# PrimeIntellect-ai/protocol

Hardware: AMD Instinct MI355X
Metric: task x worker pair-evals/sec (full-swarm match) (higher is better)
Workload: dtype u64

## Files before the change

protocol_amd/csrc/pm_device.h:

```cpp
#ifndef PM_DEVICE_H
#define PM_DEVICE_H

#include <hip/hip_runtime.h>
#include <stdint.h>

#include "pm_engine.h"

namespace pm {

static constexpr double PM_RAD = 3.14159265358979323846 / 180.0;
static constexpr uint64_t PM_KEY_NOLOC = 0x7FEFFFFFFFFFFFFFull;
static constexpr double PM_A_MAX_SAFE = 1.0 - 1.0 / 1048576.0;
static constexpr double PM_A_CHORD_MIN = 1.3e-6;
static constexpr uint32_t PM_CARVE_SLOTS = 8192;
static constexpr uint32_t PM_CARVE_PART = 64;
static constexpr uint32_t PM_CARVE_SEL_CAP = 256;
static constexpr uint32_t PM_CARVE_SLOT_BITS = 13;
static constexpr uint32_t PM_CARVE_BIG_SLOTS = 262144;
static constexpr uint32_t PM_CARVE_SLOT_BITS_BIG = 18;
static constexpr uint32_t PM_CARVE_SLOT_BITS_MEM = 21;
static constexpr double PM_TIE_BAND = 1.0 / 68719476736.0;
static constexpr double PM_TIE_BAND_BIG = 1.0 / 2147483648.0;
static constexpr double PM_TIE_BAND_MEM = 1.0 / 268435456.0;
static constexpr uint32_t PM_PROP_ROW = 96;
// ... 23 lines not shown
#define PM_STREAM_PROP_WAVES_N 4
#endif
static constexpr uint32_t PM_STREAM_PROP_WAVES = PM_STREAM_PROP_WAVES_N;
static constexpr uint32_t PM_STREAM_SLW_TREQ = PM_STREAM_TP;
static constexpr uint32_t PM_STREAM_SLW_PAY = PM_STREAM_TP + 1;
static constexpr size_t PM_STREAM_LDS_BYTES = PM_CARVE_LDS_BYTES + size_t(PM_STREAM_TP) * 4 + 128;
enum { SC_CLAIM = 0,
       SC_QUIT = 16,
       SC_DROP = 32,
       SC_ROWS = 48,
       SC_LET_BE = 53,
       SC_GAVE_UP = 49,
       SC_FINISH = 50,
       SC_FINISH_TICKET = 52,
       SC_TRACE = 51,
       SC_BATCHES = 54
};
static constexpr uint32_t PM_STREAM_TRACE_CAP = 1u << 17;
enum { SROW_NONE = 0, SROW_BITMAP = 1, SROW_WALK = 2, SROW_SWEEP = 3 };

struct CompatArgs {
  uint32_t W, n_cfgs, model_words;
  const uint32_t *flags, *gpu_count, *gpu_mem, *gpu_cls, *cpu_cores, *ram, *storage;
  const pm_config_row* cfgs;
  const pm_gpu_alt_row* alts;
  const uint32_t* model_bits;
  uint64_t* compat;
};

enum : uint32_t {
  REP_WHY = 0,
  REP_IDLE = PM_WHY_N,
  REP_GROUPS,
  REP_MEMBERS,
  REP_NO_TASK,
  REP_TASKS,
  REP_STRIDE = 16
};

struct ReportArgs {
  CompatArgs c;
  const int32_t* group_of;
  const uint32_t *g_cfg, *g_n, *g_task, *live_bits;
  uint32_t G;
  const uint64_t *tmask, *tlive;
  const uint32_t* tprefix;
  uint32_t t_lo, t_cap;
  uint32_t* out;
  uint32_t *running, *workers, *allowed;
};

struct SpreadArgs {
  const uint32_t *g_n, *g_off, *members, *slot_of_row, *small, *big;
  uint32_t n_small, n_big, W;
  const uint32_t *flags, *addr_rank;
  const double *lat, *lon, *coslat;
  pm_group_spread_row* out;
};
enum : uint32_t { SPC_GROUPS = 0, SPC_MEASURED = 1, SPC_HIST = 2, SPC_N = 2 + PM_SPREAD_BUCKETS, SPC_STRIDE = 8 };
enum : uint32_t { SPV_MAX_DIAMETER = 0, SPV_MAX_HOP = 1, SPV_SUM_DIAMETER = 2, SPV_SUM_RING = 3 };
struct SpreadCfgAcc {
  uint32_t cnt[SPC_STRIDE];
  unsigned long long v[4];
};

static constexpr uint32_t PM_NEAR_CAP = 2u * PM_NEAR_MAX_K;
struct NearArgs {
  CompatArgs c;
  const int32_t* group_of;
  const double *lat, *lon, *coslat;
  const pm_near_query* q;
  uint32_t n_q, pool, k;
  pm_near_row* rows;
  uint32_t* workers;
  double* km;
};

struct ClaimArgs {
  uint32_t R;
  const uint32_t* rows;
  const int32_t* group_of;
  const uint32_t *g_n, *g_off, *g_task;
  const uint64_t* g_id;
  uint32_t* g_task_next;
  const uint32_t* chosen;
  const uint32_t* rank_in_group;
  const uint32_t* by_rank;
  const uint64_t* t_live;
  const uint32_t* t_prefix;
  pm_assignment* table;
  uint32_t* task_col;
  pm_assignment* h_table;
  uint32_t* h_gtask;
};

struct MatchPrepArgs {
  uint32_t W, G;
  const int32_t* group_of;
  const uint32_t *g_cfg, *g_n, *g_off, *members, *addr_rank, *g_task;
  uint64_t* sel;
  uint32_t *first, *count;
  uint32_t *rank_in_group, *by_rank;
  uint32_t* g_task_next;
};

struct RowUpdateArgs {
  uint32_t n;
  const double *lat_in, *lon_in;
  const uint32_t* u32_in;
  uint32_t *flags, *gpu_count, *gpu_mem, *gpu_cls, *cpu_cores, *ram, *storage, *addr_rank, *site;
  double *lat, *lon, *coslat;
  double *ux, *uy, *uz;
};

enum { CARVE_MODE_FORM = 0, CARVE_MODE_MERGE = 1 };
enum { CARVE_STATE_RUNNING = 0, CARVE_STATE_DONE = 1, CARVE_STATE_UNCERTAIN = 2, CARVE_STATE_OVERFLOW = 3,
       CARVE_STATE_ABORTED = 4 };
enum {
  CARVE_F_INIT = 1u << 0,
  CARVE_F_RUN = 1u << 1,
  CARVE_F_ALL = 1u << 2,
  CARVE_F_PROPS = 1u << 3,
  CARVE_F_EXTPREP = 1u << 4
};
struct CarveStatus {
  uint32_t state;
  uint32_t stop_ci;
  uint32_t n_groups;
  uint32_t n_members;
  uint32_t steps_total;
  uint32_t n_eligible;
  uint32_t cur_ci;
  uint32_t n_list;
  unsigned long long cand_sum;
  uint32_t prop_k;
  uint32_t prop_limit;
  uint32_t n_seeds;
  uint32_t total_available;
  uint32_t fast_steps;
  uint32_t slow_steps;
  uint32_t n_solo;
  uint32_t n_props;
  uint32_t g_lo, g_hi;
  uint32_t n_batches;
  uint32_t n_void;
  uint32_t why[8];
  uint32_t stream_timeouts;
  uint32_t stream_tickets;
  uint32_t stream_switches;
  uint32_t stream_listed;
  uint32_t stream_pre_used;
  uint32_t stream_pre_lost;
  uint32_t stream_refreshes;
  uint32_t _pad_sr;
  uint32_t cell_g;
  uint32_t n_indexed;
  uint32_t pruned_batches;
  uint32_t prune_fallbacks;
#ifdef PM_BATCH_LOG
  uint32_t blog_n;
  uint32_t blog[3 * 512];
#endif
  unsigned long long prop_keys;
  unsigned long long prof[64];
};

struct alignas(16) BatchDesc {
  uint32_t planned;
  uint32_t ci0;
  uint32_t total_available;
  uint32_t valid;
  uint32_t none;
  uint32_t ci, n_list, prop_k, prop_limit, n_seeds;
  uint32_t cell_g;
};

struct CarveArgs {
  uint32_t mode;
  uint32_t W;
  uint32_t proximity;
  uint32_t debug_uncertain_every;
  const uint32_t* wflags;
  const double *lat, *lon, *coslat;
  const double *ux, *uy, *uz;
  const uint32_t* site;
  const uint64_t* compat;
  int32_t* group_of;
  uint32_t* order;
  uint32_t n_order;
  uint32_t _pad2;
  double *c_lat, *c_lon, *c_cos;
  double *c_ux, *c_uy, *c_uz;
  uint32_t* c_site;
  uint64_t* c_compat;
  uint64_t *alive_g, *loc_g;
  double *cc_lat, *cc_lon, *cc_cos;
  double *cc_ux, *cc_uy, *cc_uz;
  uint32_t* cc_site;
  uint32_t* slot_pos;
  uint32_t* slot_wid;
  uint64_t* bits_scratch;
  uint64_t* keys;
  uint32_t bits_stride;
  uint32_t _pad0;
  uint64_t* prop;
  uint64_t* seed_map;
  uint32_t* seed_prefix;
  uint32_t* seed_slots;
  uint32_t count_keys, _pad_ck;
  uint32_t* prep_block_counts;
  uint32_t* prep_counts;
  BatchDesc* desc;
  uint64_t* alive_snap;
  uint32_t _pad_sp;
  uint32_t debug_mem_above;
  uint32_t* cell_cnt;
  uint32_t* cell_start;
  uint32_t *pos_cell, *pos_rank;
  uint32_t* cs_of_pos;
  uint32_t* cs_slot;
  double *cs_ux, *cs_uy, *cs_uz;
  uint32_t* cs_site;
  uint32_t prune_mode;
  uint32_t prune_factor;
  uint32_t walk_cap_div, _pad_w;
  uint32_t stream, stream_tag0;
  double* c_pack;
  double* cs_pack;
  uint64_t* cfgbits;
  unsigned long long* stream_sq;
  unsigned long long* stream_row_lo;
  unsigned long long* stream_row_hi;
  uint32_t* stream_ctl;
  uint32_t stream_la, stream_row_spins;
  uint32_t stream_la_div;
  uint32_t debug_abort_after;
  unsigned long long id_state;
  uint32_t id_g0, stage_m0;
  uint32_t stage_cap_g, stage_cap_m;
  uint32_t *stage_cfg, *stage_n, *stage_off, *stage_mem;
  unsigned long long* g_id_out;
  uint32_t* g_task_out;
  CarveStatus* h_status;
  unsigned long long* stream_trace;
  uint32_t n_avail, start_ci;
  uint32_t avail_cfg[PM_MAX_CONFIGS];
  uint32_t min_size[PM_MAX_CONFIGS];
  uint32_t max_size[PM_MAX_CONFIGS];
  uint32_t *g_cfg, *g_n, *g_off, *members;
  uint32_t cap_groups, cap_members;
  CarveStatus* status;
};

void launch_compat(const CompatArgs& a, hipStream_t s);
void launch_explain(const CompatArgs& p, const uint32_t* rows, uint32_t n, uint32_t stride, uint32_t* why_out, hipStream_t s);
void launch_config_report(const ReportArgs& a, uint32_t max_blocks, hipStream_t s);
void launch_task_report(const ReportArgs& a, uint32_t max_blocks, hipStream_t s);
void launch_group_spread(const SpreadArgs& a, hipStream_t s);
void launch_config_spread(const pm_group_spread_row* rows, const uint32_t* row_cfg, uint32_t n_rows, uint32_t n_cfgs,
                          SpreadCfgAcc* out, uint32_t max_blocks, hipStream_t s);
void launch_nearest(const NearArgs& a, hipStream_t s);
void launch_geo(const double* lat, const double* lon, double* coslat, double* ux, double* uy, double* uz, uint32_t W,
                hipStream_t s);
void launch_triad(const double* b, const double* c, double* a, size_t n, hipStream_t s);
#ifdef PM_ROW_BENCH
hipError_t launch_row_bench(const CarveArgs* d_args, uint32_t seed, uint32_t ci, uint32_t reps, uint32_t mode, unsigned long long* d_out, hipStream_t s);
#endif
void launch_row_network_test(const uint64_t* keys, const uint32_t* sites, uint32_t n_waves, uint32_t n_per_wave, uint32_t slot_bits,
                             uint64_t ulps, uint32_t upto, uint64_t* rows_out, uint32_t* mismatches, hipStream_t s);
static constexpr uint32_t PM_DK_WORDS = 20;
void launch_distance_key_test(const double* in, const double* geo, uint32_t n, uint32_t mode, double* out, hipStream_t s);
void launch_update_rows(const RowUpdateArgs& a, hipStream_t s);
void launch_worker_selector(const int32_t* group_of, const uint32_t* g_cfg, uint32_t R, const uint32_t* rows,
                            uint64_t* sel, hipStream_t s);
void launch_eligible_selector(const uint32_t* wflags, const int32_t* group_of, const uint64_t* compat,
                              uint64_t enabled, uint32_t W, const uint8_t* shard, uint32_t my_rank, uint64_t* sel,
                              hipStream_t s);
void launch_chooser_rank(const int32_t* group_of, const uint64_t* g_id, const uint32_t* count, uint32_t R,
                         const uint32_t* rows, uint64_t seed, uint32_t* rank, hipStream_t s);
void launch_table_scatter(const pm_assignment* x, const uint32_t* xrow, uint32_t W, pm_assignment* table,
                          uint32_t* task_col, uint32_t* g_task_next, const uint64_t* t_live, const uint32_t* t_prefix,
                          hipStream_t s);
void launch_group_rank(const int32_t* group_of, const uint32_t* g_n, const uint32_t* g_off, const uint32_t* members,
                       const uint32_t* addr_rank, uint32_t W, uint32_t* rank_in_group, uint32_t* by_rank,
                       hipStream_t s);
void launch_claim_publish(const ClaimArgs& a, hipStream_t s);
void launch_match_prep(const MatchPrepArgs& a, hipStream_t s);
void launch_build_planes(const uint64_t* col_mask, uint32_t n_cols, uint32_t c_begin, uint32_t c_end, uint32_t stride,
                         uint32_t n_planes, uint64_t* planes, hipStream_t s);
void launch_pair_sweep(int variant, const uint64_t* row_sel, uint32_t R, const uint64_t* col_mask,
                       const uint64_t* planes, uint32_t c_begin, uint32_t c_end, uint32_t stride, uint32_t n_planes,
                       uint32_t* first, uint32_t* count, hipStream_t s, bool inited = false);
void launch_pair_select(int variant, const uint64_t* row_sel, uint32_t R, const uint64_t* col_mask,
                        const uint64_t* planes, uint32_t c_begin, uint32_t c_end, uint32_t stride, uint32_t n_planes,
                        const uint32_t* rank, uint32_t* out, hipStream_t s);
void launch_task_prefix(const uint64_t* live, uint32_t w_begin, uint32_t w_end, uint32_t* prefix, hipStream_t s);
void launch_task_delete(const uint32_t* slots, uint32_t n, uint64_t* tmask, uint64_t* live, uint64_t* planes,
                        uint32_t stride, uint32_t n_planes, hipStream_t s);
void launch_task_intern(const uint64_t* tmask, const uint64_t* live, uint32_t u_begin, uint32_t u_end, uint64_t valid,
                        uint64_t* keys, uint32_t n_slots, uint32_t* vals, uint32_t* counter_and_overflow, uint64_t* umask,
                        uint32_t cap_u, hipStream_t s);
void launch_task_compact_class(const uint32_t* first_c, const uint32_t* count_c, const uint64_t* tmask, uint64_t valid,
                               const uint64_t* keys, const uint32_t* vals, uint32_t n_slots, uint32_t u_begin,
                               uint32_t u_end, const uint64_t* live, const uint32_t* prefix, uint32_t* first_out,
                               uint32_t* count_out, hipStream_t s);
void launch_task_compact(const uint32_t* first_u, const uint32_t* count_u, uint32_t u_begin, uint32_t u_end,
                         const uint64_t* live, const uint32_t* prefix, uint32_t* first_out, uint32_t* count_out,
                         hipStream_t s);
void launch_newest(const int64_t* created_at, const uint64_t* live, uint32_t t_begin, uint32_t t_end,
                   uint32_t* idx_by_block, long long* val_by_block, uint32_t n_blocks, hipStream_t s);
void launch_group_ids(uint64_t* g_id, uint32_t* g_task, uint32_t n, uint64_t rng_state, hipStream_t s);
hipError_t carve_kernels_init();
hipError_t launch_carve(const CarveArgs* d_args, uint32_t flags, uint32_t start_ci, size_t lds_bytes, hipStream_t s);
uint32_t launch_carve_prep(const CarveArgs* d_args, uint32_t W, hipStream_t s);
hipError_t launch_carve_args_put(const CarveArgs& a, CarveArgs* d_args, hipStream_t s);
uint32_t launch_carve_elig(CarveArgs* d_args, const CarveArgs* put, uint32_t W, uint32_t n_bound, uint32_t index_min, uint32_t start_ci,
                           bool fresh, uint32_t n_groups0, uint32_t n_members0, hipStream_t s);
void launch_carve_apply(const CarveArgs* d_args, uint32_t W, hipStream_t s);
void launch_carve_propose(const CarveArgs* d_args, uint32_t W, hipStream_t s);
hipError_t launch_carve_stream(const CarveArgs* d_args, uint32_t start_ci, uint32_t n_prop_wgs, hipStream_t s);
void launch_scatter_const(uint32_t* dst, const uint32_t* idx, uint32_t n, uint32_t v, hipStream_t s);
void launch_scatter_pairs(uint32_t* dst, const uint32_t* pairs, uint32_t n, hipStream_t s);
void launch_merge_place(const CarveArgs* d_args, uint32_t n_order, uint32_t n_groups0, uint32_t n_members0, uint32_t steps0,
                        hipStream_t s);

}
#endif
```

protocol_amd/csrc/pm_engine.cpp:

```cpp
#include <hip/hip_runtime.h>

#include <algorithm>
#include <atomic>
#include <cmath>
#include <chrono>
#include <cstdio>
#include <cstdlib>
#include <cstring>
#include <functional>
#include <memory>
#include <mutex>
#include <string>
#include <thread>
#include <unordered_map>
#include <vector>

#include "pm_device.h"
#include "pm_engine.h"
#include "pm_internal.h"
#include "pm_members.h"

namespace pm {

static thread_local std::string g_last_error;

int32_t set_error(int32_t code, const std::string& msg) {
  g_last_error = msg;
  return code;
}

#define HIPCHK(expr)                                                                                   \
  do {                                                                                                 \
    hipError_t e_ = (expr);                                                                            \
    if (e_ != hipSuccess)                                                                              \
      return set_error(PM_ENODEV, std::string(#expr) + ": " + hipGetErrorString(e_));                  \
  } while (0)

#include "pm_engine_types.inc"
}

using namespace pm;

namespace pm {
struct FormRun;
}

#include "pm_engine_state.inc"

namespace pm {

#include "pm_engine_groups.inc"
#include "pm_engine_carve.inc"
#include "pm_engine_match.inc"
#include "pm_engine_merge.inc"
}


extern "C" {

const char* pm_last_error(void) { return pm::g_last_error.c_str(); }

void pm_engine_config_default(pm_engine_config* c) {
  if (!c) return;
  std::memset(c, 0, sizeof(*c));
  c->abi_version = PM_ABI_VERSION;
  c->device = 0;
  c->proximity_enabled = 1;
  c->switching_enabled = 1;
  c->prefer_larger_groups = 1;
  c->chooser = PM_CHOOSE_FIRST;
  c->group_id_seed = 1;
}

int32_t pm_engine_create(const pm_engine_config* cfg, pm_engine** out) {
  if (!cfg || !out) return set_error(PM_EINVAL, "null argument");
  if (cfg->abi_version != PM_ABI_VERSION) return set_error(PM_EINVAL, "ABI version mismatch");
  if (cfg->carve_variant != 0 && cfg->carve_variant != 1 && cfg->carve_variant != 3)
    return set_error(PM_EINVAL, "carve_variant: 0 (streaming carve), 1 (exact sweep only) or 3 (batch pipeline); 2 and 4 were removed");
  int n_dev = 0;
  if (hipGetDeviceCount(&n_dev) != hipSuccess || n_dev <= 0)
    return set_error(PM_ENODEV, "no HIP device visible: the matching engine needs an MI355X (gfx950); there is no CPU fallback");
  if (cfg->device < 0 || cfg->device >= n_dev) return set_error(PM_EINVAL, "device ordinal out of range");
  HIPCHK(hipSetDevice(cfg->device));
  hipDeviceProp_t prop;
  HIPCHK(hipGetDeviceProperties(&prop, cfg->device));
  if (std::strncmp(prop.gcnArchName, "gfx950", 6) != 0)
    return set_error(PM_ENODEV, std::string("device is ") + prop.gcnArchName + ", kernels are built for gfx950 only");
  HIPCHK(carve_kernels_init());
  pm_engine* e = new (std::nothrow) pm_engine();
  if (!e) return set_error(PM_ENOMEM, "out of host memory");
  e->cfg = *cfg;
  e->id_rng = cfg->group_id_seed;
  if (const char* v = getenv("PM_PRUNE_MODE")) {
    if (v[0] >= '0' && v[0] <= '3' && !v[1]) e->prune_mode = uint32_t(v[0] - '0');
  }
  if (const char* v = getenv("PM_WALK_CAP_DIV")) {
    const long f = atol(v);
    if (f > 0 && f < 1000) e->walk_cap_div = uint32_t(f);
  }
  if (const char* v = getenv("PM_PRUNE_FACTOR")) {
    const long f = atol(v);
    if (f > 0 && f < (1l << 30)) e->prune_factor = uint32_t(f);
  }
  if (const char* v = getenv("PM_STREAM_WGS")) {
    const long f = atol(v);
    if (f > 0 && f < 4096) e->stream_wgs_env = uint32_t(f);
  }
  if (const char* v = getenv("PM_STREAM_ROW_SPINS")) {
    const long f = atol(v);
    if (f > 0 && f < (1l << 24)) e->stream_row_spins_env = uint32_t(f);
  }
  if (const char* v = getenv("PM_STREAM_LA_DIV")) {
    const long f = atol(v);
    if (f > 0 && f < 4096) e->stream_la_div_env = uint32_t(f);
  }
  if (const char* v = getenv("PM_MERGE_STREAM_MIN")) {
    const long f = atol(v);
    if (f >= 2 && f <= (1l << 30)) e->merge_stream_min = uint32_t(f);
  }
  if (const char* v = getenv("PM_STREAM_LA")) {
    const long f = atol(v);
    if (f > 0 && f <= long(PM_STREAM_LA_MAX)) e->stream_la_env = uint32_t(f);
  }
  {
    int cus = 0;
    if (hipDeviceGetAttribute(&cus, hipDeviceAttributeMultiprocessorCount, cfg->device) == hipSuccess && cus > 0)
      e->n_cus = uint32_t(cus);
  }
  if (hipStreamCreateWithFlags(&e->stream, hipStreamNonBlocking) != hipSuccess) {
    delete e;
    return set_error(PM_ENODEV, "hipStreamCreate failed");
  }
  e->stream_owned = e->stream;
  for (auto& ev : e->ev)
    if (hipEventCreate(&ev) != hipSuccess) {
      delete e;
      return set_error(PM_ENODEV, "hipEventCreate failed");
    }
  for (auto& ev : e->kev)
    if (hipEventCreate(&ev) != hipSuccess) {
      delete e;
      return set_error(PM_ENODEV, "hipEventCreate failed");
    }
  if (hipEventCreateWithFlags(&e->ev_groups, hipEventDisableTiming) != hipSuccess) {
    delete e;
    return set_error(PM_ENODEV, "hipEventCreate failed");
  }
  *out = e;
  return PM_OK;
}

void pm_engine_destroy(pm_engine* e) {
  if (!e) return;
  (void)hipSetDevice(e->cfg.device);
  (void)hipStreamSynchronize(e->stream);
  e->d_cfgs.release(); e->d_alts.release(); e->d_model_bits.release();
  e->d_flags.release(); e->d_gpu_count.release(); e->d_gpu_mem.release(); e->d_gpu_cls.release();
  e->d_cpu_cores.release(); e->d_ram.release(); e->d_storage.release(); e->d_addr_rank.release();
  e->d_lat.release(); e->d_lon.release(); e->d_coslat.release(); e->d_compat.release();
  e->d_ux.release(); e->d_uy.release(); e->d_uz.release();
  for (int k = 0; k < 3; ++k) { e->d_c_u[k].release(); e->d_cc_u[k].release(); }
  e->d_tmask.release(); e->d_tplanes.release(); e->d_created.release(); e->d_tlive.release(); e->d_tprefix.release();
  e->d_first_c.release(); e->d_count_c.release(); e->d_tdel.release();
  e->d_group_of.release(); e->d_g_cfg.release(); e->d_g_n.release(); e->d_g_off.release();
  e->d_g_task.release(); e->d_g_task_next.release(); e->d_members.release(); e->d_by_rank.release();
  e->d_rank_in_group.release(); e->d_g_id.release();
  e->d_order.release(); e->d_c_lat.release(); e->d_c_lon.release(); e->d_c_cos.release();
  e->d_cc_lat.release(); e->d_cc_lon.release(); e->d_cc_cos.release(); e->d_slot_pos.release(); e->d_slot_wid.release();
  e->d_site.release(); e->d_c_site.release(); e->d_cc_site.release(); e->d_prop.release(); e->d_seed_map.release(); e->d_seed_prefix.release(); e->d_seed_slots.release(); e->d_prep_block_counts.release(); e->d_prep_counts.release();
  e->d_c_compat.release(); e->d_keys.release(); e->d_bits.release(); e->d_status.release(); e->d_carve_args.release();
  e->d_m_cfg.release(); e->d_m_n.release(); e->d_m_off.release(); e->d_m_members.release();
  e->d_cfgbits.release(); e->d_stream_sq.release(); e->d_stream_row_lo.release(); e->d_stream_row_hi.release();
  e->d_stream_ctl.release(); e->d_stream_trace.release();
  e->d_sel.release(); e->d_wplanes.release(); e->d_sel_perm.release();
  e->d_first.release(); e->d_count.release(); e->d_rank.release(); e->d_chosen.release(); e->d_perm.release();
  e->d_table.release(); e->d_task_col.release(); e->d_shard.release(); e->d_own_rows.release(); e->d_xrow.release();
  e->d_sel_own.release(); e->d_table_x.release(); e->d_row_stage.release(); if (e->h_row_pin) (void)hipHostFree(e->h_row_pin); if (e->ev_row_stage) (void)hipEventDestroy(e->ev_row_stage); e->d_nb_idx.release(); e->d_nb_val.release();
  if (e->h_gstage) (void)hipHostFree(e->h_gstage);
  if (e->h_status) (void)hipHostFree(e->h_status);
  for (int k = 0; k < 2; ++k) {
    if (e->h_delta_pin[k]) (void)hipHostFree(e->h_delta_pin[k]);
    e->d_delta[k].release();
  }
  if (e->h_gtask_pinned) (void)hipHostFree(e->h_gtask_pinned);
  if (e->ev_groups) (void)hipEventDestroy(e->ev_groups);
  for (PubTable& t : e->pub)
    if (t.words.load()) (void)hipHostFree(t.words.load());
  for (uint64_t* q : e->pub_retired) (void)hipHostFree(q);
  for (auto& ev : e->ev)
    if (ev) (void)hipEventDestroy(ev);
  for (auto& ev : e->kev)
    if (ev) (void)hipEventDestroy(ev);
  for (hipEvent_t x : e->prop_ev) (void)hipEventDestroy(x);
  if (e->stream_owned) (void)hipStreamDestroy(e->stream_owned);
  e->d_cell_cnt.release(); e->d_cell_start.release(); e->d_pos_cell.release(); e->d_pos_rank.release();
  e->d_cs_of_pos.release(); e->d_cs_slot.release(); e->d_cs_site.release();
  for (auto& u : e->d_cs_u) u.release();
  e->d_c_pack.release();
  e->d_cs_pack.release();
  e->d_desc.release(); e->d_snap.release(); e->d_ikeys.release(); e->d_umask.release(); e->d_ivals.release();
  e->d_rep_rows.release(); e->d_rep_why.release(); e->d_rep_flags.release(); e->d_rep_live.release(); e->d_rep_g.release();
  e->d_rep_tprefix.release(); e->d_rep_cnt.release(); e->d_rep_task.release(); e->d_rep_gof.release();
  e->d_spr_idx.release(); e->d_spr_rows.release(); e->d_spr_acc.release();
  e->d_near_q.release(); e->d_near_out.release();
  delete e->form;
  delete e;
}

int32_t pm_set_configs(pm_engine* e, const pm_config_row* cfgs, uint32_t n_cfgs, const pm_gpu_alt_row* alts,
                       uint32_t n_alts) {
  if (!e || (n_cfgs && !cfgs) || (n_alts && !alts)) return set_error(PM_EINVAL, "null argument");
  if (n_cfgs > PM_MAX_CONFIGS) return set_error(PM_EINVAL, "more than PM_MAX_CONFIGS configurations");
  for (uint32_t i = 0; i < n_cfgs; ++i) {
    if (cfgs[i].max_group_size < cfgs[i].min_group_size)
      return set_error(PM_EINVAL, "Plugin configuration is invalid (max_group_size < min_group_size)");
    if (cfgs[i].min_group_size == 0)
      return set_error(PM_EINVAL, "min_group_size == 0 is rejected (the reference would form empty groups forever)");
    if (uint64_t(cfgs[i].alt_begin) + cfgs[i].alt_count > n_alts)
      return set_error(PM_ERANGE, "alternative range outside the alt table");
  }
  std::lock_guard<std::mutex> lk(e->mu);
  if (e->dist_phase != 0) return set_error(PM_ESTATE, "a stepwise tick is in progress");
  HIPCHK(hipSetDevice(e->cfg.device));
  e->cfgs.assign(cfgs, cfgs + n_cfgs);
  e->alts.assign(alts, alts + n_alts);
  int32_t rc = upload(e->d_cfgs, e->cfgs.data(), e->cfgs.size(), e->stream);
  if (rc) return rc;
  rc = upload(e->d_alts, e->alts.data(), e->alts.size(), e->stream);
  if (rc) return rc;
  HIPCHK(e->d_model_bits.ensure(1));
  HIPCHK(hipStreamSynchronize(e->stream));
  e->have_cfgs = true;
  e->compat_dirty = true;
  e->tplanes_dirty = true;
  return PM_OK;
}

int32_t pm_set_model_table(pm_engine* e, const uint32_t* bits, uint32_t n_rows, uint32_t n_classes) {
  if (!e || (n_rows && n_classes && !bits)) return set_error(PM_EINVAL, "null argument");
  std::lock_guard<std::mutex> lk(e->mu);
  HIPCHK(hipSetDevice(e->cfg.device));
  const size_t words = size_t(n_rows) * ((n_classes + 31u) / 32u);
  e->model_bits.assign(bits, bits + words);
  e->model_rows = n_rows;
  e->model_classes = n_classes;
  e->cls_check_dirty = true;
  int32_t rc = upload(e->d_model_bits, e->model_bits.data(), words, e->stream);
  if (rc) return rc;
  HIPCHK(hipStreamSynchronize(e->stream));
  e->compat_dirty = true;
  return PM_OK;
}

int32_t pm_set_enabled_mask(pm_engine* e, uint64_t enabled) {
  if (!e) return set_error(PM_EINVAL, "null argument");
  std::lock_guard<std::mutex> lk(e->mu);
  if (e->dist_phase != 0) return set_error(PM_ESTATE, "a stepwise tick is in progress");
  e->enabled = enabled;
  return PM_OK;
}

#include "pm_engine_workers.inc"
#include "pm_engine_tasks.inc"
// ... 10 lines not shown
```

protocol_amd/csrc/pm_engine_carve.inc:

```
static int32_t ensure_compat(pm_engine* e, hipEvent_t end_ev = nullptr) {
  if (!e->have_cfgs || !e->have_workers) return set_error(PM_ESTATE, "configs and workers must be uploaded first");
  {
    int32_t rcf = sync_flags(e);
    if (rcf) return rcf;
  }
  if (!e->compat_dirty) return PM_OK;
  for (const pm_gpu_alt_row& a : e->alts)
    if ((a.flags & PM_G_MODEL) && a.model_row >= e->model_rows)
      return set_error(PM_ESTATE, "a GPU alternative names a model row but pm_set_model_table was not called");
  if (e->model_rows && e->cls_check_dirty)
    for (uint32_t w = 0; w < e->W; ++w)
      if ((e->h_flags[w] & PM_W_GPU_MODEL) && e->h_gpu_cls[w] >= e->model_classes)
        return set_error(PM_ERANGE, "worker gpu_model_class outside the model table");
  e->cls_check_dirty = false;
  HIPCHK(e->d_compat.ensure(std::max<size_t>(e->W, 1)));
  CompatArgs a{};
  a.W = e->W;
  a.n_cfgs = uint32_t(e->cfgs.size());
  a.model_words = (e->model_classes + 31u) / 32u;
  a.flags = e->d_flags.p;
  a.gpu_count = e->d_gpu_count.p;
  a.gpu_mem = e->d_gpu_mem.p;
  a.gpu_cls = e->d_gpu_cls.p;
  a.cpu_cores = e->d_cpu_cores.p;
// ... 50 lines not shown
  HIPCHK(e->d_c_lat.ensure(cap));
  HIPCHK(e->d_c_lon.ensure(cap));
  HIPCHK(e->d_c_cos.ensure(cap));
  HIPCHK(e->d_cc_lat.ensure(cap));
  HIPCHK(e->d_cc_lon.ensure(cap));
  HIPCHK(e->d_cc_cos.ensure(cap));
  for (int k = 0; k < 3; ++k) {
    HIPCHK(e->d_c_u[k].ensure(cap));
    HIPCHK(e->d_cc_u[k].ensure(cap));
  }
  HIPCHK(e->d_c_compat.ensure(cap));
  HIPCHK(e->d_keys.ensure(cap));
  HIPCHK(e->d_slot_pos.ensure(cap));
  HIPCHK(e->d_slot_wid.ensure(cap));
  HIPCHK(e->d_c_site.ensure(cap));
  HIPCHK(e->d_cc_site.ensure(cap));
  {
    HIPCHK(e->d_prop.ensure((size_t(PM_PROP_MAX_SEEDS) + 64) * PM_PROP_ROW));
    HIPCHK(e->d_seed_map.ensure((cap + 63) / 64 + 64));
    HIPCHK(e->d_seed_prefix.ensure((cap + 63) / 64 + 64));
    HIPCHK(e->d_seed_slots.ensure(size_t(PM_PROP_MAX_SEEDS) + 128));
    HIPCHK(e->d_prep_block_counts.ensure(((cap + 255) / 256 + 1) * PM_MAX_CONFIGS));
    HIPCHK(e->d_prep_counts.ensure(PM_MAX_CONFIGS + 8));
  }
  HIPCHK(e->d_status.ensure(1));
  HIPCHK(e->d_carve_args.ensure(1));
  HIPCHK(e->d_desc.ensure(1));
  const uint32_t stride = uint32_t((cap + 63) / 64);
  HIPCHK(e->d_bits.ensure(size_t(stride) * 4));
  HIPCHK(e->d_snap.ensure(stride));
  if (stream) {
    HIPCHK(e->d_c_pack.ensure(cap * 4));
    HIPCHK(e->d_cs_pack.ensure(cap * 4));
    HIPCHK(e->d_cfgbits.ensure(size_t(stride) * PM_MAX_CONFIGS));
    HIPCHK(e->d_stream_ctl.ensure(PM_STREAM_CTL_WORDS));
    if (!e->d_stream_sq.p) {
      HIPCHK(e->d_stream_sq.ensure(PM_STREAM_SQ));
      HIPCHK(e->d_stream_row_lo.ensure(size_t(PM_STREAM_RQ) * 64));
      HIPCHK(e->d_stream_row_hi.ensure(size_t(PM_STREAM_RQ) * 64));
      e->stream_seq = 0;
    }
  }
  if (mode == CARVE_MODE_FORM && e->prune_mode && e->cfg.proximity_enabled) {
    if (!e->d_cell_cnt.p) {
      HIPCHK(e->d_cell_cnt.ensure(PM_CELL_TABLE));
      HIPCHK(hipMemsetAsync(e->d_cell_cnt.p, 0, e->d_cell_cnt.cap * sizeof(uint32_t), e->stream));
    }
    if (!e->d_cell_start.p) {
      HIPCHK(e->d_cell_start.ensure(PM_CELL_TABLE + 384));
      HIPCHK(hipMemsetAsync(e->d_cell_start.p, 0, e->d_cell_start.cap * sizeof(uint32_t), e->stream));
    }
    HIPCHK(e->d_pos_cell.ensure(cap));
    HIPCHK(e->d_pos_rank.ensure(cap));
    HIPCHK(e->d_cs_of_pos.ensure(cap));
    HIPCHK(e->d_cs_slot.ensure(cap));
    HIPCHK(e->d_cs_site.ensure(cap));
    for (auto& u : e->d_cs_u) HIPCHK(u.ensure(cap));
  }
  std::memset(a, 0, sizeof(*a));
  a->mode = mode;
  a->W = e->W;
  a->proximity = e->cfg.proximity_enabled;
  a->debug_uncertain_every = e->cfg.debug_uncertain_every;
  a->wflags = e->d_flags.p;
  a->lat = e->d_lat.p;
  a->lon = e->d_lon.p;
  a->coslat = e->d_coslat.p;
  a->ux = e->d_ux.p;
  a->uy = e->d_uy.p;
  a->uz = e->d_uz.p;
  a->compat = e->d_compat.p;
  a->group_of = e->d_group_of.p;
  a->order = e->d_order.p;
  a->n_order = n_order;
  a->c_lat = e->d_c_lat.p;
  a->c_lon = e->d_c_lon.p;
  a->c_cos = e->d_c_cos.p;
  a->c_ux = e->d_c_u[0].p;
  a->c_uy = e->d_c_u[1].p;
  a->c_uz = e->d_c_u[2].p;
  a->c_compat = e->d_c_compat.p;
  a->alive_g = e->d_bits.p;
  a->loc_g = e->d_bits.p + stride;
  a->cc_lat = e->d_cc_lat.p;
  a->cc_lon = e->d_cc_lon.p;
  a->cc_cos = e->d_cc_cos.p;
  a->cc_ux = e->d_cc_u[0].p;
  a->cc_uy = e->d_cc_u[1].p;
  a->cc_uz = e->d_cc_u[2].p;
  a->keys = e->d_keys.p;
  a->slot_pos = e->d_slot_pos.p;
  a->slot_wid = e->d_slot_wid.p;
  a->site = e->d_site.p;
  a->c_site = e->d_c_site.p;
  a->cc_site = e->d_cc_site.p;
  a->prop = e->d_prop.p;
  a->seed_map = e->d_seed_map.p;
  a->seed_prefix = e->d_seed_prefix.p;
  a->seed_slots = e->d_seed_slots.p;
  a->count_keys = e->cfg.time_proposer ? 1u : 0u;
  a->prep_block_counts = e->d_prep_block_counts.p;
  a->prep_counts = e->d_prep_counts.p;
  a->bits_scratch = e->d_bits.p + size_t(stride) * 2;
  a->bits_stride = stride;
  a->status = e->d_status.p;
  a->desc = e->d_desc.p;
  a->alive_snap = e->d_snap.p;
  a->debug_mem_above = e->debug_mem_above;
  if (mode == CARVE_MODE_FORM && e->prune_mode && e->cfg.proximity_enabled) {
    a->prune_mode = e->prune_mode;
    a->prune_factor = e->prune_factor;
    a->walk_cap_div = e->walk_cap_div;
    a->cell_cnt = e->d_cell_cnt.p;
    a->cell_start = e->d_cell_start.p;
    a->pos_cell = e->d_pos_cell.p;
    a->pos_rank = e->d_pos_rank.p;
    a->cs_of_pos = e->d_cs_of_pos.p;
    a->cs_slot = e->d_cs_slot.p;
    a->cs_site = e->d_cs_site.p;
    a->cs_ux = e->d_cs_u[0].p;
    a->cs_uy = e->d_cs_u[1].p;
    a->cs_uz = e->d_cs_u[2].p;
  }
  if (stream) {
    a->stream = 1;
    a->cc_lat = a->c_lat;
    a->cc_lon = a->c_lon;
    a->cc_cos = a->c_cos;
    a->cc_ux = a->c_ux;
    a->cc_uy = a->c_uy;
    a->cc_uz = a->c_uz;
    a->cc_site = a->c_site;
    a->slot_wid = a->order;
    a->bits_scratch = e->d_bits.p;
    a->loc_g = e->d_bits.p + stride;
    a->alive_g = e->d_bits.p + size_t(stride) * 2;
    a->cfgbits = e->d_cfgbits.p;
    a->c_pack = e->d_c_pack.p;
    a->cs_pack = e->d_cs_pack.p;
    a->stream_sq = (unsigned long long*)e->d_stream_sq.p;
    a->stream_row_lo = (unsigned long long*)e->d_stream_row_lo.p;
    a->stream_row_hi = (unsigned long long*)e->d_stream_row_hi.p;
    a->stream_ctl = e->d_stream_ctl.p;
#if defined(PM_CARVE_PROF) || defined(PM_ROW_REC)
    HIPCHK(e->d_stream_trace.ensure(size_t(PM_STREAM_TRACE_CAP) * 2));
    a->stream_trace = (unsigned long long*)e->d_stream_trace.p;
#endif
#ifdef PM_ROW_REC
    HIPCHK(hipMemsetAsync(e->d_stream_trace.p, 0, size_t(PM_STREAM_TRACE_CAP) * 16, e->stream));
#endif
    a->stream_la = e->stream_la_env;
    a->stream_la_div = e->stream_la_div_env;
    a->stream_row_spins = e->stream_row_spins_env;
    a->debug_abort_after = e->debug_abort_after;
  }
  return PM_OK;
}

static int32_t host_resolve_form_step(pm_engine* e, uint32_t cfg, CarveStatus* st) {
  int32_t rc = pull_compat(e);
  if (rc) return rc;
  std::vector<int32_t> group_of(e->W);
  if (e->W) {
    HIPCHK(hipMemcpyAsync(group_of.data(), e->d_group_of.p, size_t(e->W) * 4, hipMemcpyDeviceToHost, e->stream));
    HIPCHK(hipStreamSynchronize(e->stream));
  }
  const pm_config_row& c = e->cfgs[cfg];
  std::vector<uint32_t> compat;
  size_t total_available = 0;
  for (uint32_t w = 0; w < e->W; ++w) {
    const uint32_t f = e->h_flags[w];
    if (!((f & PM_W_HEALTHY) && (f & PM_W_HAS_P2P) && group_of[w] < 0)) continue;
    ++total_available;
    if ((e->h_compat[w] >> cfg) & 1ull) compat.push_back(w);
  }
  if (total_available < c.min_group_size || compat.size() < c.min_group_size || compat.empty())
    return set_error(PM_ESTATE, "host resolve: nothing to carve (state mismatch)");
  uint32_t seed = compat[0];
  bool seed_loc = false;
  for (uint32_t w : compat)
    if (e->h_flags[w] & PM_W_HAS_LOC) {
      seed = w;
      seed_loc = true;
      break;
    }
  std::vector<uint32_t> rest;
  for (uint32_t w : compat)
    if (w != seed) rest.push_back(w);
  if (seed_loc && e->cfg.proximity_enabled) {
    std::vector<double> d(e->W, 0.0);
    for (uint32_t w : rest)
      d[w] = (e->h_flags[w] & PM_W_HAS_LOC) ? host_distance(e->h_lat[seed], e->h_lon[seed], e->h_lat[w], e->h_lon[w])
                                            : 1.7976931348623157e308;
    std::stable_sort(rest.begin(), rest.end(), [&](uint32_t a, uint32_t b) { return d[a] < d[b]; });
  }
  std::vector<uint32_t> members{seed};
  for (uint32_t w : rest) {
    if (members.size() >= c.max_group_size) break;
    members.push_back(w);
  }
  if (members.size() < c.min_group_size) return set_error(PM_ESTATE, "host resolve: group below min size");
  const uint32_t g = st->n_groups, off = st->n_members, n = uint32_t(members.size());
  if (g >= e->d_g_cfg.cap || off + n > e->d_members.cap) return set_error(PM_ENOMEM, "group arrays overflow");
  HIPCHK(hipMemcpyAsync(e->d_g_cfg.p + g, &cfg, 4, hipMemcpyHostToDevice, e->stream));
  HIPCHK(hipMemcpyAsync(e->d_g_n.p + g, &n, 4, hipMemcpyHostToDevice, e->stream));
  HIPCHK(hipMemcpyAsync(e->d_g_off.p + g, &off, 4, hipMemcpyHostToDevice, e->stream));
  HIPCHK(hipMemcpyAsync(e->d_members.p + off, members.data(), size_t(n) * 4, hipMemcpyHostToDevice, e->stream));
  for (uint32_t w : members) group_of[w] = int32_t(g);
  HIPCHK(hipMemcpyAsync(e->d_group_of.p, group_of.data(), size_t(e->W) * 4, hipMemcpyHostToDevice, e->stream));
  HIPCHK(hipStreamSynchronize(e->stream));
  st->n_groups += 1;
  st->n_members += n;
  st->n_solo += n == 1 ? 1u : 0u;
  st->steps_total += 1;
  return PM_OK;
}

static int32_t absorb_groups(pm_engine* e) {
  if (!e->absorb_pending) return PM_OK;
  HIPCHK(hipEventSynchronize(e->ev_groups));
  const uint32_t g0 = e->ab_g0, ng = e->ab_g1 - e->ab_g0, m0 = e->ab_m0;
  const uint32_t *g_cfg = e->ab_cfg_p, *g_n = e->ab_n_p, *g_off = e->ab_off_p, *members = e->ab_mem_p;
  if (e->groups.capacity() < e->groups.size() + ng) e->groups.reserve(std::max(e->groups.size() + ng, e->groups.capacity() * 2));
  for (uint32_t k = 0; k < ng; ++k) {
    Group gr;
    gr.id = splitmix64_next(&e->id_rng);
    gr.cfg = g_cfg[k];
    gr.task = PM_NONE;
    gr.task_uid = 0;
    gr.members.assign(members + (g_off[k] - m0), members + (g_off[k] - m0) + g_n[k]);
    for (uint32_t w : gr.members) e->h_group_of[w] = int32_t(g0 + k);
    log_group_event(e, PM_GROUP_CREATED, gr);
    e->groups.push_back(std::move(gr));
  }
  e->absorb_pending = false;
  return PM_OK;
}

#define ABSORB_PENDING(e)                 \
  do {                                    \
    int32_t rc_abs_ = absorb_groups(e);   \
    if (rc_abs_) return rc_abs_;          \
  } while (0)

static void host_mark(const char* what) {
  static const bool on = [] { const char* v = getenv("PM_TRACE_HOST"); return v && *v == '1'; }();
  if (!on) return;
  static const auto t0 = std::chrono::steady_clock::now();
  const double us = std::chrono::duration<double, std::micro>(std::chrono::steady_clock::now() - t0).count();
  fprintf(stderr, "[pm host] %10.1f us  %s\n", us, what);
}

struct FormRun {
  CarveArgs a;
  CarveStatus st;
  std::vector<uint32_t> avail;
  uint32_t g0 = 0, m0 = 0, start_ci = 0;
  size_t lds = 0;
  bool use_props = false;
  bool nothing = false;
  uint32_t n_bound = 0;
  uint32_t n_elig_hint = 0;
  bool stream = false;
  uint32_t stream_wgs = 0;
  bool rearmed = false;
  uint32_t stage_cap = 0;
  bool args_pending = false;
};

static int32_t launch_propose_timed(pm_engine* e, const CarveArgs* d_args, uint32_t n_bound, hipStream_t s);

static int32_t form_setup_args(pm_engine* e, FormRun* r);

static int32_t form_queue_init(pm_engine* e, FormRun* r, bool fresh = false) {
  fresh = fresh && r->use_props;
  if (!fresh) HIPCHK(hipMemcpyAsync(e->d_status.p, &r->st, sizeof(r->st), hipMemcpyHostToDevice, e->stream));
  if (r->use_props) {
    if (!r->stream) HIPCHK(hipMemsetAsync(e->d_desc.p, 0, sizeof(BatchDesc), e->stream));
    const uint32_t index_min = !r->a.prune_mode ? 0u : r->a.prune_mode >= 2u ? 1u : PM_CELL_AUTO_N;
    if (r->stream) {
      if (e->stream_seq == 0 || e->stream_seq >= 127) {
        HIPCHK(hipMemsetAsync(e->d_stream_sq.p, 0, size_t(PM_STREAM_SQ) * 8, e->stream));
        HIPCHK(hipMemsetAsync(e->d_stream_row_lo.p, 0, size_t(PM_STREAM_RQ) * 64 * 8, e->stream));
        HIPCHK(hipMemsetAsync(e->d_stream_row_hi.p, 0, size_t(PM_STREAM_RQ) * 64 * 8, e->stream));
        e->stream_seq = 0;
      }
      e->stream_seq += 1;
      const uint32_t tag0 = e->stream_seq << 25;
      if (r->a.stream_tag0 != tag0) {
        r->a.stream_tag0 = tag0;
        if (!r->args_pending)
          HIPCHK(hipMemcpyAsync(&e->d_carve_args.p->stream_tag0, &r->a.stream_tag0, sizeof(uint32_t), hipMemcpyHostToDevice, e->stream));
      }
    }
    e->tick_carve_launches += launch_carve_elig(e->d_carve_args.p, r->args_pending ? &r->a : nullptr, e->W, r->n_bound,
                                                r->n_elig_hint >= index_min ? index_min : 0u, r->start_ci, fresh, r->st.n_groups,
                                                r->st.n_members, e->stream);
    r->args_pending = false;
    host_mark("form: eligible list queued");
    if (r->stream) {
      HIPCHK(launch_carve_stream(e->d_carve_args.p, r->start_ci, r->stream_wgs, e->stream));
      e->tick_carve_launches += 2;
      return PM_OK;
    }
    e->tick_carve_launches += launch_carve_prep(e->d_carve_args.p, r->n_bound, e->stream);
    HIPCHK(hipGetLastError());
  } else
    HIPCHK(launch_carve(e->d_carve_args.p, CARVE_F_INIT | CARVE_F_RUN | CARVE_F_ALL, r->start_ci, r->lds, e->stream));
  e->tick_carve_launches++;
  return PM_OK;
}

static int32_t form_begin(pm_engine* e, FormRun* r, hipEvent_t begin_ev = nullptr) {
  int32_t rc = absorb_groups(e);
  if (rc) return rc;
  rc = ensure_compat(e);
  if (rc) return rc;
  rc = push_groups(e);
  if (rc) return rc;
  available_order(e->cfgs.data(), uint32_t(e->cfgs.size()), e->enabled, &r->avail);
  r->g0 = e->d_n_groups;
  r->m0 = e->d_n_members;
  r->start_ci = 0;
  r->nothing = r->avail.empty() || e->W == 0;
  if (r->nothing) return PM_OK;
  if (e->h_group_of.size() == e->W && e->h_flags.size() == e->W) {
    const int32_t* const gof = e->h_group_of.data();
    const uint32_t* const fl = e->h_flags.data();
    const uint32_t need = PM_W_HEALTHY | PM_W_HAS_P2P;
    uint32_t nb = 0, ne = 0;
    for (uint32_t w = 0; w < e->W; ++w) {
      const uint32_t un = uint32_t(gof[w]) >> 31;
      nb += un;
      ne += un & uint32_t((fl[w] & need) == need);
    }
    r->n_bound = nb;
    r->n_elig_hint = ne;
  } else {
    r->n_bound = uint32_t(std::count_if(e->h_group_of.begin(), e->h_group_of.end(), [](int32_t g) { return g < 0; }));
    r->n_elig_hint = r->n_bound;
  }
  if (e->h_group_of.size() != e->W) r->n_bound = r->n_elig_hint = e->W;
  if (r->n_bound == 0) r->n_bound = 1;
  r->st = CarveStatus{};
  r->st.state = CARVE_STATE_RUNNING;
  r->st.n_groups = r->g0;
  r->st.n_members = r->m0;
  r->use_props = e->cfg.carve_variant != 1 && e->cfg.proximity_enabled;
  r->stream = r->use_props && e->cfg.carve_variant == 0 && r->n_bound <= PM_CARVE_BIG_SLOTS &&
              !e->debug_mem_above;
  host_mark("form: begin (host mirrors counted)");
  rc = form_setup_args(e, r);
  if (rc) return rc;
  host_mark("form: arguments queued");
  if (begin_ev && r->args_pending) {
    e->k_carve_begin = begin_ev;
  } else {
    HIPCHK(hipEventRecord(e->kev[2], e->stream));
    e->k_carve_begin = e->kev[2];
  }
  return form_queue_init(e, r, true);
}

static int32_t form_setup_args(pm_engine* e, FormRun* r) {
  CarveArgs& a = r->a;
  int32_t rc = fill_carve_args(e, &a, CARVE_MODE_FORM, 0, r->stream);
  if (rc) return rc;
  if (r->stream) {
    uint32_t wgs = e->stream_wgs_env ? e->stream_wgs_env : r->n_elig_hint / 64u + 48u;
    const uint32_t max_wgs = e->n_cus > 8u ? e->n_cus - 4u : 4u;
    r->stream_wgs = std::max(1u, std::min(wgs, max_wgs));
    a.stream_tag0 = ((e->stream_seq == 0 || e->stream_seq >= 127) ? 1u : e->stream_seq + 1u) << 25;
    a.id_state = e->id_rng;
    a.id_g0 = r->g0;
    a.stage_m0 = r->m0;
    a.g_id_out = (unsigned long long*)e->d_g_id.p;
    a.g_task_out = e->d_g_task.p;
    r->stage_cap = std::max<uint32_t>(r->n_bound, 1u);
    const size_t need = size_t(4) * r->stage_cap;
    if (e->h_gstage_cap < need) {
      HIPCHK(hipStreamSynchronize(e->stream));
      if (e->h_gstage) (void)hipHostFree(e->h_gstage);
      e->h_gstage = nullptr;
      e->h_gstage_cap = 0;
      const size_t cap = std::max<size_t>(need, size_t(4) * std::max<uint32_t>(e->W, 1));
      HIPCHK(hipHostMalloc((void**)&e->h_gstage, cap * sizeof(uint32_t)));
      e->h_gstage_cap = cap;
    }
    if (!e->h_status) HIPCHK(hipHostMalloc((void**)&e->h_status, sizeof(CarveStatus)));
    a.stage_cap_g = a.stage_cap_m = r->stage_cap;
    a.stage_cfg = e->h_gstage;
    a.stage_n = e->h_gstage + r->stage_cap;
    a.stage_off = e->h_gstage + size_t(2) * r->stage_cap;
    a.stage_mem = e->h_gstage + size_t(3) * r->stage_cap;
    a.h_status = e->h_status;
    e->h_status->state = 0xFFFFFFFFu;
  }
  a.n_avail = uint32_t(r->avail.size());
  for (size_t i = 0; i < r->avail.size(); ++i) {
    a.avail_cfg[i] = r->avail[i];
    a.min_size[i] = e->cfgs[r->avail[i]].min_group_size;
    a.max_size[i] = e->cfgs[r->avail[i]].max_group_size;
  }
  a.g_cfg = e->d_g_cfg.p;
  a.g_n = e->d_g_n.p;
  a.g_off = e->d_g_off.p;
  a.members = e->d_members.p;
  a.cap_groups = uint32_t(std::min<size_t>(e->d_g_cfg.cap, 0xFFFFFFFFu));
  a.cap_members = uint32_t(std::min<size_t>(e->d_members.cap, 0xFFFFFFFFu));
  bool in_lds;
  r->lds = carve_lds_bytes(a.bits_stride, &in_lds);
  r->args_pending = r->use_props;
  if (!r->args_pending) HIPCHK(launch_carve_args_put(a, e->d_carve_args.p, e->stream));
  return PM_OK;
}

static int32_t launch_propose_timed(pm_engine* e, const CarveArgs* d_args, uint32_t n_bound, hipStream_t s) {
  if (!e->cfg.time_proposer) {
    launch_carve_propose(d_args, n_bound, s);
    return PM_OK;
  }
  while (e->prop_ev.size() < e->prop_ev_used + 2) {
    hipEvent_t x = nullptr;
    HIPCHK(hipEventCreate(&x));
    e->prop_ev.push_back(x);
  }
  HIPCHK(hipEventRecord(e->prop_ev[e->prop_ev_used], s));
  launch_carve_propose(d_args, n_bound, s);
  HIPCHK(hipEventRecord(e->prop_ev[e->prop_ev_used + 1], s));
  e->prop_ev_used += 2;
  return PM_OK;
}

static int32_t form_queue_pairs(pm_engine* e, FormRun* r, uint32_t count) {
  for (uint32_t k = 0; k < count; ++k) {
    int32_t rc = launch_propose_timed(e, e->d_carve_args.p, r->n_bound, e->stream);
    if (rc) return rc;
    HIPCHK(launch_carve(e->d_carve_args.p, CARVE_F_RUN | CARVE_F_PROPS | CARVE_F_EXTPREP, 0, r->lds, e->stream));
    e->tick_carve_launches += 2u + launch_carve_prep(e->d_carve_args.p, r->n_bound, e->stream);
  }
  return PM_OK;
}

static int32_t form_poll(pm_engine* e, FormRun* r) {
  for (;;) {
    HIPCHK(hipEventRecord(e->kev[3], e->stream));
    HIPCHK(hipMemcpyAsync(&r->st, e->d_status.p, sizeof(r->st), hipMemcpyDeviceToHost, e->stream));
    HIPCHK(hipStreamSynchronize(e->stream));
    {
      float ms = 0;
      HIPCHK(hipEventElapsedTime(&ms, e->k_carve_begin ? e->k_carve_begin : e->kev[2], e->kev[3]));
      e->k_ms_carve += ms;
      HIPCHK(hipEventRecord(e->kev[2], e->stream));
      e->k_carve_begin = e->kev[2];
      for (size_t k = 0; k + 1 < e->prop_ev_used; k += 2) {
        HIPCHK(hipEventElapsedTime(&ms, e->prop_ev[k], e->prop_ev[k + 1]));
        e->k_ms_propose += ms;
      }
      e->prop_ev_used = 0;
    }
    if (r->st.state == CARVE_STATE_OVERFLOW) return set_error(PM_ENOMEM, "carve: group arrays overflow");
    if (r->st.state == CARVE_STATE_ABORTED) {
      if (!r->stream) return set_error(PM_ENODEV, "carve: a hand-shake inside the validator timed out");
      e->tick_stream_aborts++;
      r->rearmed = true;
      r->stream = false;
      int32_t rca = form_setup_args(e, r);
      if (rca) return rca;
      r->start_ci = r->st.stop_ci;
      r->st.state = CARVE_STATE_RUNNING;
      rca = form_queue_init(e, r);
      if (rca) return rca;
      return PM_OK;
    }
    if (r->st.state != CARVE_STATE_UNCERTAIN) return PM_OK;
    int32_t rc = host_resolve_form_step(e, r->avail[r->st.stop_ci], &r->st);
    if (rc) return rc;
    e->tick_host_resolved++;
    r->rearmed = true;
    r->start_ci = r->st.stop_ci;
    r->st.state = CARVE_STATE_RUNNING;
    rc = form_queue_init(e, r);
    if (rc) return rc;
  }
}

static int32_t form_finish(pm_engine* e, FormRun* r, uint32_t* n_formed, bool defer_absorb, bool have_event = false) {
  if (n_formed) *n_formed = 0;
  if (r->nothing) return PM_OK;
  const CarveStatus& st = r->st;
  e->tick_fast_steps += st.fast_steps;
  e->tick_carve_steps += st.steps_total;
  e->tick_cand_sum += st.cand_sum;
  e->tick_props += r->stream && !st.n_props ? st.stream_tickets : st.n_props;
  e->tick_prop_keys += st.prop_keys;
  e->tick_stream_timeouts += st.stream_timeouts;
  e->tick_stream_tickets += st.stream_tickets;
  std::memcpy(e->carve_prof, st.prof, sizeof(st.prof));
  for (int k = 0; k < 8; ++k) e->carve_why[k] = st.why[k];
  e->carve_why[8] = st.n_batches;
  e->carve_why[9] = st.n_void;
  e->carve_why[10] = st.pruned_batches;
  e->carve_why[11] = st.prune_fallbacks;
  e->carve_why[12] = st.cell_g;
  e->carve_why[13] = st.n_indexed;
  e->carve_why[14] = r->stream ? 1u : 0u;
  e->carve_why[15] = st.stream_tickets;
  e->carve_why[16] = st.stream_timeouts;
  e->carve_why[17] = st.stream_switches;
  e->carve_why[18] = st.stream_listed;
  e->carve_why[19] = r->stream_wgs;
  e->carve_why[20] = e->tick_stream_aborts;
  e->carve_why[21] = st.slow_steps;
  e->carve_why[22] = st.stream_pre_used;
  e->carve_why[23] = st.stream_pre_lost;
  e->carve_why[24] = st.stream_refreshes;
#ifdef PM_BATCH_LOG
  e->blog.assign(st.blog, st.blog + 3 * std::min<uint32_t>(st.blog_n, 512u));
#endif

  const uint32_t g0 = r->g0, m0 = r->m0, g1 = st.n_groups, m1 = st.n_members;
  if (g1 > g0) {
    const uint32_t ng = g1 - g0, nm = m1 - m0;
    const bool staged = r->stream && !r->rearmed && ng <= r->stage_cap && nm <= r->stage_cap;
    if (staged) {
      e->ab_cfg_p = e->h_gstage;
      e->ab_n_p = e->h_gstage + r->stage_cap;
      e->ab_off_p = e->h_gstage + size_t(2) * r->stage_cap;
      e->ab_mem_p = e->h_gstage + size_t(3) * r->stage_cap;
      if (!have_event) HIPCHK(hipEventRecord(e->ev_groups, e->stream));
    } else {
      const size_t need = size_t(3) * ng + nm;
      if (e->h_gstage_cap < need) {
        if (e->h_gstage) (void)hipHostFree(e->h_gstage);
        e->h_gstage = nullptr;
        e->h_gstage_cap = 0;
        const size_t cap = std::max<size_t>(need, size_t(4) * std::max<uint32_t>(e->W, 1));
        HIPCHK(hipHostMalloc((void**)&e->h_gstage, cap * sizeof(uint32_t)));
        e->h_gstage_cap = cap;
      }
      uint32_t* st_cfg = e->h_gstage;
      HIPCHK(hipMemcpyAsync(st_cfg, e->d_g_cfg.p + g0, size_t(ng) * 4, hipMemcpyDeviceToHost, e->stream));
      HIPCHK(hipMemcpyAsync(st_cfg + ng, e->d_g_n.p + g0, size_t(ng) * 4, hipMemcpyDeviceToHost, e->stream));
      HIPCHK(hipMemcpyAsync(st_cfg + 2 * size_t(ng), e->d_g_off.p + g0, size_t(ng) * 4, hipMemcpyDeviceToHost, e->stream));
      HIPCHK(hipMemcpyAsync(st_cfg + 3 * size_t(ng), e->d_members.p + m0, size_t(nm) * 4, hipMemcpyDeviceToHost, e->stream));
      e->ab_cfg_p = st_cfg;
      e->ab_n_p = st_cfg + ng;
      e->ab_off_p = st_cfg + 2 * size_t(ng);
      e->ab_mem_p = st_cfg + 3 * size_t(ng);
      HIPCHK(hipEventRecord(e->ev_groups, e->stream));
      host_mark("form: group copies queued");
      launch_group_ids(e->d_g_id.p + g0, e->d_g_task.p + g0, ng, e->id_rng, e->stream);
      HIPCHK(hipGetLastError());
    }
    e->absorb_pending = true;
    e->ab_g0 = g0;
    e->ab_g1 = g1;
    e->ab_m0 = m0;
    e->ab_m1 = m1;
    e->ab_solo = st.n_solo;
    e->d_n_groups = g1;
    e->d_n_members = m1;
    if (!defer_absorb) {
      int32_t rc = absorb_groups(e);
      if (rc) return rc;
    }
  }
  if (n_formed) *n_formed = g1 - g0;
  return PM_OK;
}

static int32_t run_form_wait(pm_engine* e, FormRun& r) {
  int32_t rc = PM_OK;
  if (!r.nothing) {
    uint32_t batch = e->form_rounds_hint ? e->form_rounds_hint + 1u : r.a.n_avail + 3u;
    for (uint32_t spins = 0;; ++spins) {
      if (spins > 4096u + e->W / 8u) return set_error(PM_ENODEV, "carve made no progress");
      if (r.use_props && !r.stream) {
        rc = form_queue_pairs(e, &r, batch);
        if (rc) return rc;
      }
      host_mark("form: carve queued");
      rc = form_poll(e, &r);
      if (rc) return rc;
      host_mark("form: status back");
      if (r.st.state == CARVE_STATE_DONE) break;
      if (r.st.state != CARVE_STATE_RUNNING || !r.use_props) return set_error(PM_ENODEV, "carve kernel did not complete");
      if (r.stream) return set_error(PM_ENODEV, "streaming carve did not complete");
      batch = 8u;
    }
  }
  if (!r.nothing && r.use_props && !r.stream) e->form_rounds_hint = r.st.n_batches + r.st.n_void;
  return PM_OK;
}
static int32_t run_form_rest(pm_engine* e, FormRun& r, uint32_t* n_formed, bool defer_absorb) {
  int32_t rc = run_form_wait(e, r);
  if (rc) return rc;
  return form_finish(e, &r, n_formed, defer_absorb);
}

static int32_t run_form(pm_engine* e, uint32_t* n_formed, bool defer_absorb = false) {
  FormRun r;
  int32_t rc = form_begin(e, &r);
  if (rc) return rc;
  return run_form_rest(e, r, n_formed, defer_absorb);
}
```

protocol_amd/csrc/pm_engine_debug.inc:

```
int32_t pm_debug_carve_prof(pm_engine* e, unsigned long long* out, uint32_t cap) {
  if (!e || !out) return set_error(PM_EINVAL, "null argument");
  std::lock_guard<std::mutex> lk(e->mu);
  const uint32_t n = std::min<uint32_t>(cap, 32u);
  std::memcpy(out, e->carve_prof, size_t(n) * sizeof(unsigned long long));
  for (uint32_t k = 32; k < cap && k < 56; ++k) out[k] = e->carve_why[k - 32];
  for (uint32_t k = 56; k < cap && k < 88; ++k) out[k] = e->carve_prof[k - 56 + 32];
  const unsigned long long inc[9] = {e->t_lo, e->t_cap, e->T, e->t_dead, e->t_regrowths, e->t_compactions,
                                     e->groups.size(), e->n_dead_groups, e->pub_retired.size()};
  for (uint32_t k = 88; k < cap && k < 97; ++k) out[k] = inc[k - 88];
  if (cap > 97u) out[97] = e->carve_why[24];
  return PM_OK;
}

int32_t pm_debug_stream_trace(pm_engine* e, unsigned long long* out, uint32_t cap, uint32_t* n) {
  if (!e || !out || !n) return set_error(PM_EINVAL, "null argument");
  std::lock_guard<std::mutex> lk(e->mu);
  *n = 0;
  if (!e->d_stream_trace.p || !e->d_stream_ctl.p) return PM_OK;
  uint32_t cnt = 0;
  HIPCHK(hipMemcpy(&cnt, e->d_stream_ctl.p + SC_TRACE, 4, hipMemcpyDeviceToHost));
#ifdef PM_ROW_REC
  cnt = std::min<uint32_t>(cnt, std::min<uint32_t>(cap, PM_STREAM_TRACE_CAP / 8u));
  if (cnt) HIPCHK(hipMemcpy(out, e->d_stream_trace.p + PM_STREAM_TRACE_CAP, size_t(cnt) * 16, hipMemcpyDeviceToHost));
#else
  cnt = std::min<uint32_t>(cnt, std::min<uint32_t>(cap, PM_STREAM_TRACE_CAP));
  if (cnt) HIPCHK(hipMemcpy(out, e->d_stream_trace.p, size_t(cnt) * 16, hipMemcpyDeviceToHost));
#endif
  *n = cnt;
  return PM_OK;
}

int32_t pm_debug_row_records(pm_engine* e, unsigned long long* out, uint32_t cap_rows, uint32_t* n_rows) {
  if (!e || !out || !n_rows) return set_error(PM_EINVAL, "null argument");
  std::lock_guard<std::mutex> lk(e->mu);
  *n_rows = 0;
#ifdef PM_ROW_REC
  if (!e->d_stream_trace.p) return PM_OK;
  const uint32_t n = std::min<uint32_t>(cap_rows, PM_STREAM_TRACE_CAP / 8u);
  HIPCHK(hipMemcpy(out, e->d_stream_trace.p, size_t(n) * 64, hipMemcpyDeviceToHost));
  *n_rows = n;
#endif
  return PM_OK;
}
int32_t pm_debug_chain_batches(pm_engine* e, unsigned long long* out, uint32_t cap, uint32_t* n) {
  if (!e || !out || !n) return set_error(PM_EINVAL, "null argument");
  std::lock_guard<std::mutex> lk(e->mu);
  *n = 0;
#ifdef PM_ROW_REC
  if (!e->d_stream_trace.p || !e->d_stream_ctl.p) return PM_OK;
  uint32_t cnt = 0;
  HIPCHK(hipMemcpy(&cnt, e->d_stream_ctl.p + SC_BATCHES, 4, hipMemcpyDeviceToHost));
  cnt = std::min<uint32_t>(cnt, std::min<uint32_t>(cap, PM_STREAM_TRACE_CAP / 8u));
  if (cnt) HIPCHK(hipMemcpy(out, e->d_stream_trace.p + PM_STREAM_TRACE_CAP + PM_STREAM_TRACE_CAP / 2u, size_t(cnt) * 32, hipMemcpyDeviceToHost));
  *n = cnt;
#endif
  return PM_OK;
}
int32_t pm_debug_park_records(pm_engine* e, unsigned long long* out, uint32_t cap_blocks, uint32_t* n_blocks) {
  if (!e || !out || !n_blocks) return set_error(PM_EINVAL, "null argument");
  std::lock_guard<std::mutex> lk(e->mu);
  *n_blocks = 0;
#ifdef PM_ROW_REC
  if (!e->d_stream_trace.p) return PM_OK;
  const uint32_t n = std::min<uint32_t>(cap_blocks, PM_STREAM_TRACE_CAP / 32u);
  HIPCHK(hipMemcpy(out, e->d_stream_trace.p + PM_STREAM_TRACE_CAP + PM_STREAM_TRACE_CAP / 4u, size_t(n) * 64, hipMemcpyDeviceToHost));
  *n_blocks = n;
#endif
  return PM_OK;
}
int32_t pm_debug_mem_lists_above(pm_engine* e, uint32_t n) {
  if (!e) return set_error(PM_EINVAL, "null argument");
  std::lock_guard<std::mutex> lk(e->mu);
  e->debug_mem_above = n;
  return PM_OK;
}

int32_t pm_debug_stream_abort_after(pm_engine* e, uint32_t n) {
  if (!e) return set_error(PM_EINVAL, "null argument");
  std::lock_guard<std::mutex> lk(e->mu);
  e->debug_abort_after = n;
  return PM_OK;
}

int32_t pm_debug_merge_streamed(pm_engine* e, uint32_t* n) {
  if (!e || !n) return set_error(PM_EINVAL, "null argument");
  std::lock_guard<std::mutex> lk(e->mu);
  *n = e->merge_streamed;
  return PM_OK;
}

int32_t pm_debug_delta_pushes(pm_engine* e, uint32_t* n) {
  if (!e || !n) return set_error(PM_EINVAL, "null argument");
  std::lock_guard<std::mutex> lk(e->mu);
  *n = e->delta_pushes;
  return PM_OK;
}

int32_t pm_debug_prune_mode(pm_engine* e, uint32_t mode) {
  if (!e || mode > 3u) return set_error(PM_EINVAL, "prune mode 0..3");
  std::lock_guard<std::mutex> lk(e->mu);
  e->prune_mode = mode;
  return PM_OK;
}

#ifdef PM_BATCH_LOG
extern "C" int32_t pm_debug_batch_log(pm_engine* e, uint32_t* out, uint32_t cap_words, uint32_t* n_words) {
  if (!e || !out || !n_words) return set_error(PM_EINVAL, "null argument");
  std::lock_guard<std::mutex> lk(e->mu);
  *n_words = uint32_t(e->blog.size());
  std::memcpy(out, e->blog.data(), sizeof(uint32_t) * std::min<size_t>(cap_words, e->blog.size()));
  return PM_OK;
}
#endif

int32_t pm_debug_hbm_triad(pm_engine* e, uint64_t n_doubles, uint32_t reps, double* gb_per_s) {
  if (!e || !gb_per_s || !n_doubles) return set_error(PM_EINVAL, "null argument");
  std::lock_guard<std::mutex> lk(e->mu);
  HIPCHK(hipSetDevice(e->cfg.device));
  double *a = nullptr, *b = nullptr, *c = nullptr;
  HIPCHK(hipMalloc((void**)&a, n_doubles * 8));
  if (hipMalloc((void**)&b, n_doubles * 8) != hipSuccess || hipMalloc((void**)&c, n_doubles * 8) != hipSuccess) {
    (void)hipFree(a);
    if (b) (void)hipFree(b);
    return set_error(PM_ENOMEM, "triad buffers");
  }
  (void)hipMemsetAsync(b, 0, n_doubles * 8, e->stream);
  (void)hipMemsetAsync(c, 0, n_doubles * 8, e->stream);
  float best = 1e30f;
  for (uint32_t r = 0; r < reps + 1; ++r) {
    (void)hipEventRecord(e->kev[0], e->stream);
    launch_triad(b, c, a, size_t(n_doubles), e->stream);
    (void)hipEventRecord(e->kev[1], e->stream);
    (void)hipEventSynchronize(e->kev[1]);
    float ms = 0;
    (void)hipEventElapsedTime(&ms, e->kev[0], e->kev[1]);
    if (r > 0 && ms < best) best = ms;
  }
  (void)hipFree(a);
  (void)hipFree(b);
  (void)hipFree(c);
  *gb_per_s = double(n_doubles) * 24.0 / (double(best) * 1e-3) / 1e9;
  return PM_OK;
}

int32_t pm_debug_row_networks(pm_engine* e, const uint64_t* keys, const uint32_t* sites, uint32_t n_waves, uint32_t n_per_wave,
                              uint32_t slot_bits, uint64_t ulps, uint32_t upto, uint64_t* rows_out, uint32_t* mismatches) {
  if (!e || !keys || !sites || !rows_out || !mismatches || !n_waves || (n_waves & 3u) || !n_per_wave || slot_bits == 0 || slot_bits > 24)
    return set_error(PM_EINVAL, "null argument");
  std::lock_guard<std::mutex> lk(e->mu);
  HIPCHK(hipSetDevice(e->cfg.device));
  const size_t nk = size_t(n_waves) * n_per_wave, ns = size_t(1) << slot_bits;
  uint64_t *d_k = nullptr, *d_rows = nullptr;
  uint32_t *d_s = nullptr, *d_m = nullptr;
  int32_t rc = PM_OK;
  if (hipMalloc((void**)&d_k, nk * 8) != hipSuccess || hipMalloc((void**)&d_rows, size_t(n_waves) * 64 * 8) != hipSuccess ||
      hipMalloc((void**)&d_s, ns * 4) != hipSuccess || hipMalloc((void**)&d_m, 8) != hipSuccess) {
    rc = set_error(PM_ENOMEM, "row network test buffers");
  } else {
    (void)hipMemcpyAsync(d_k, keys, nk * 8, hipMemcpyHostToDevice, e->stream);
    (void)hipMemcpyAsync(d_s, sites, ns * 4, hipMemcpyHostToDevice, e->stream);
    (void)hipMemsetAsync(d_m, 0, 8, e->stream);
    launch_row_network_test(d_k, d_s, n_waves, n_per_wave, slot_bits, ulps, upto, d_rows, d_m, e->stream);
    (void)hipMemcpyAsync(rows_out, d_rows, size_t(n_waves) * 64 * 8, hipMemcpyDeviceToHost, e->stream);
    (void)hipMemcpyAsync(mismatches, d_m, 8, hipMemcpyDeviceToHost, e->stream);
    if (hipStreamSynchronize(e->stream) != hipSuccess) rc = set_error(PM_ENODEV, "row network test");
  }
  if (d_k) (void)hipFree(d_k);
  if (d_rows) (void)hipFree(d_rows);
  if (d_s) (void)hipFree(d_s);
  if (d_m) (void)hipFree(d_m);
  return rc;
}

int32_t pm_debug_distance_keys(pm_engine* e, const double* in, uint32_t n, uint32_t mode, double* out) {
  if (!e || !out || mode > 2u) return set_error(PM_EINVAL, "null argument");
  if (mode == 2u) {
    const double c[8] = {PM_A_CHORD_MIN, PM_A_MAX_SAFE, PM_TIE_BAND, PM_TIE_BAND_BIG, PM_TIE_BAND_MEM,
                         double(PM_CARVE_SLOT_BITS), double(PM_CARVE_SLOT_BITS_BIG), double(PM_CARVE_SLOT_BITS_MEM)};
    std::memcpy(out, c, sizeof(c));
    return PM_OK;
  }
  if (!in || n == 0 || n > (1u << 26)) return set_error(PM_EINVAL, "distance keys: 1 to 2^26 inputs");
  std::lock_guard<std::mutex> lk(e->mu);
  HIPCHK(hipSetDevice(e->cfg.device));
  const size_t n_in = mode == 0u ? size_t(5) * n : n, n_out = mode == 0u ? size_t(PM_DK_WORDS) * n : n;
  double *d_in = nullptr, *d_geo = nullptr, *d_out = nullptr;
  int32_t rc = PM_OK;
  if (hipMalloc((void**)&d_in, n_in * 8) != hipSuccess || hipMalloc((void**)&d_out, n_out * 8) != hipSuccess ||
      (mode == 0u && hipMalloc((void**)&d_geo, size_t(8) * n * 8) != hipSuccess)) {
    rc = set_error(PM_ENOMEM, "distance key test buffers");
  } else {
    (void)hipMemcpyAsync(d_in, in, n_in * 8, hipMemcpyHostToDevice, e->stream);
    if (mode == 0u)
      launch_geo(d_in, d_in + size_t(2) * n, d_geo, d_geo + size_t(2) * n, d_geo + size_t(4) * n, d_geo + size_t(6) * n, 2u * n,
                 e->stream);
    launch_distance_key_test(d_in, d_geo, n, mode, d_out, e->stream);
    (void)hipMemcpyAsync(out, d_out, n_out * 8, hipMemcpyDeviceToHost, e->stream);
    if (hipStreamSynchronize(e->stream) != hipSuccess) rc = set_error(PM_ENODEV, "distance key test");
  }
  if (d_in) (void)hipFree(d_in);
  if (d_geo) (void)hipFree(d_geo);
  if (d_out) (void)hipFree(d_out);
  return rc;
}

#ifdef PM_ROW_BENCH
extern "C" int32_t pm_debug_row_bench(pm_engine* e, uint32_t ci, uint32_t kth, uint32_t reps, uint32_t mode, unsigned long long* out) {
  if (!e || !out) return set_error(PM_EINVAL, "null argument");
  std::lock_guard<std::mutex> lk(e->mu);
  HIPCHK(hipSetDevice(e->cfg.device));
  if (!e->d_carve_args.p) return set_error(PM_ESTATE, "no match yet");
  CarveArgs h;
  HIPCHK(hipMemcpy(&h, e->d_carve_args.p, sizeof(h), hipMemcpyDeviceToHost));
  if (!h.cfgbits || !h.bits_stride || ci >= h.n_avail) return set_error(PM_ESTATE, "no configuration bitmaps");
  std::vector<uint64_t> row(h.bits_stride);
  HIPCHK(hipMemcpy(row.data(), h.cfgbits + size_t(ci) * h.bits_stride, h.bits_stride * 8, hipMemcpyDeviceToHost));
  uint32_t seed = PM_NONE, seen = 0;
  for (size_t j = 0; j < row.size() && seed == PM_NONE; ++j)
    for (uint64_t w = row[j]; w; w &= w - 1)
      if (seen++ == kth) {
        seed = uint32_t(j * 64 + __builtin_ctzll(w));
        break;
      }
  if (seed == PM_NONE) return set_error(PM_EINVAL, "fewer candidates than that");
  unsigned long long *d_ones = nullptr, *d_out = nullptr;
  CarveArgs* d_h = nullptr;
  int32_t rc = PM_OK;
  if (hipMalloc((void**)&d_ones, h.bits_stride * 8) != hipSuccess || hipMalloc((void**)&d_out, 64) != hipSuccess ||
      hipMalloc((void**)&d_h, sizeof(h)) != hipSuccess) {
    rc = set_error(PM_ENOMEM, "row bench buffers");
  } else {
    (void)hipMemset(d_ones, 0xFF, h.bits_stride * 8);
    (void)hipMemset(d_out, 0, 64);
    h.bits_scratch = (uint64_t*)d_ones;
    (void)hipMemcpy(d_h, &h, sizeof(h), hipMemcpyHostToDevice);
    if (launch_row_bench(d_h, seed, ci, reps, mode, d_out, e->stream) != hipSuccess || hipStreamSynchronize(e->stream) != hipSuccess)
      rc = set_error(PM_ENODEV, "row bench");
    else
      (void)hipMemcpy(out, d_out, 64, hipMemcpyDeviceToHost);
    out[7] = seed;
  }
  if (d_ones) (void)hipFree(d_ones);
  if (d_out) (void)hipFree(d_out);
  if (d_h) (void)hipFree(d_h);
  return rc;
}
#endif

int32_t pm_last_stats(pm_engine* e, pm_stats* stats) {
  if (!e || !stats) return set_error(PM_EINVAL, "null argument");
  std::lock_guard<std::mutex> lk(e->mu);
  *stats = e->last_stats;
  return PM_OK;
}
```

protocol_amd/csrc/pm_engine_merge.inc:

```

static bool hex_id_less(uint64_t a, uint64_t b) {
  auto len = [](uint64_t x) {
    int n = 1;
    while (x >>= 4) ++n;
    return n;
  };
  const int la = len(a), lb = len(b);
  const uint64_t aa = a << (4 * (16 - la)), bb = b << (4 * (16 - lb));
  if (aa != bb) return aa < bb;
  return la < lb;
}

static void host_merge_select(pm_engine* e, const std::vector<uint32_t>& rem, const pm_config_row& c,
                              std::vector<uint32_t>* batch) {
  batch->clear();
  if (e->cfg.proximity_enabled) {
    size_t seed_pos = rem.size();
    for (size_t i = 0; i < rem.size(); ++i)
      if (e->h_flags[rem[i]] & PM_W_HAS_LOC) {
        seed_pos = i;
        break;
      }
    if (seed_pos < rem.size()) {
      const uint32_t seed = rem[seed_pos];
      batch->push_back(seed);
      std::vector<std::pair<double, uint32_t>> others;
      for (size_t i = 0; i < rem.size(); ++i)
        if (i != seed_pos && (e->h_flags[rem[i]] & PM_W_HAS_LOC))
          others.emplace_back(host_distance(e->h_lat[seed], e->h_lon[seed], e->h_lat[rem[i]], e->h_lon[rem[i]]), rem[i]);
      std::stable_sort(others.begin(), others.end(), [](const auto& x, const auto& y) { return x.first < y.first; });
      for (const auto& o : others)
        if (batch->size() + 1 <= c.max_group_size) {
          batch->push_back(o.second);
          if (batch->size() >= c.max_group_size) break;
        }
    }
  }
  if (batch->empty() || (batch->size() < c.max_group_size && batch->size() < c.min_group_size)) {
    if (batch->size() < c.min_group_size) batch->clear();
    for (uint32_t w : rem) {
      if (std::find(batch->begin(), batch->end(), w) != batch->end()) continue;
      if (batch->size() + 1 <= c.max_group_size) {
        batch->push_back(w);
        if (batch->size() >= c.max_group_size) break;
      }
    }
  }
}

static int32_t run_merge(pm_engine* e, uint32_t* n_merged) {
  if (n_merged) *n_merged = 0;
  if (!e->have_cfgs || !e->have_workers) return set_error(PM_ESTATE, "configs and workers must be uploaded first");
  size_t solo = e->absorb_pending ? e->ab_solo : 0;
  for (const Group& g : e->groups) solo += g.members.size() == 1 && !g.dead;
  e->tick_needs_merge = solo >= 2;
  if (solo < 2) return PM_OK;
  {
    int32_t rc0 = absorb_groups(e);
    if (rc0) return rc0;
  }
  compact_groups(e);
  int32_t rc = ensure_compat(e);
  if (rc) return rc;
  rc = pull_compat(e);
  if (rc) return rc;
  std::vector<uint32_t> avail;
  available_order(e->cfgs.data(), uint32_t(e->cfgs.size()), e->enabled, &avail);
  uint32_t merged = 0;
  std::vector<uint8_t> used(std::max<size_t>(e->W, 1), 0);
  std::vector<uint32_t> slots, rem, order, b_n, b_off, mem;
  std::vector<std::vector<uint32_t>> batches;
  CarveArgs a;
  CarveStatus st{}, st_in{};
  for (uint32_t cfg : avail) {
    const pm_config_row& c = e->cfgs[cfg];
    compact_groups(e);
    slots.clear();
    for (uint32_t s = 0; s < e->groups.size(); ++s)
      if (e->groups[s].members.size() == 1 && ((e->h_compat[e->groups[s].members[0]] >> cfg) & 1ull)) slots.push_back(s);
    if (slots.size() < c.min_group_size) continue;
    std::sort(slots.begin(), slots.end(),
              [&](uint32_t x, uint32_t y) { return hex_id_less(e->groups[x].id, e->groups[y].id); });
    rem.clear();
    for (uint32_t s : slots) rem.push_back(e->groups[s].members[0]);

    batches.clear();
    {
      rc = push_groups(e);
      if (rc) return rc;
      order = rem;
      auto mark_used = [&](const std::vector<uint32_t>& b) {
        for (uint32_t w : b) used[w] = 1;
      };
      auto drop_used = [&]() {
        order.clear();
        for (uint32_t w : rem)
          if (!used[w]) order.push_back(w);
      };
      const size_t cap = std::max<size_t>(e->W, 1);
      HIPCHK(e->d_m_cfg.ensure(cap));
      HIPCHK(e->d_m_n.ensure(cap));
      HIPCHK(e->d_m_off.ensure(cap));
      HIPCHK(e->d_m_members.ensure(cap));
      bool try_stream = e->cfg.carve_variant == 0 && e->cfg.proximity_enabled && !e->debug_mem_above &&
                        order.size() >= e->merge_stream_min && order.size() <= PM_CARVE_BIG_SLOTS && c.max_group_size > 1 &&
                        c.max_group_size - 1u < PM_PROP_KMAX && c.min_group_size >= 1;
      for (;;) {
        const bool stream_now = try_stream;
        try_stream = false;
        rc = fill_carve_args(e, &a, CARVE_MODE_MERGE, uint32_t(order.size()), stream_now);
        if (rc) return rc;
        a.n_avail = 1;
        a.avail_cfg[0] = cfg;
        a.min_size[0] = c.min_group_size;
        a.max_size[0] = c.max_group_size;
        a.g_cfg = e->d_m_cfg.p;
        a.g_n = e->d_m_n.p;
        a.g_off = e->d_m_off.p;
        a.members = e->d_m_members.p;
        a.cap_groups = uint32_t(cap);
        a.cap_members = uint32_t(cap);
        bool in_lds;
        const size_t lds = carve_lds_bytes(a.bits_stride, &in_lds);
        st_in = CarveStatus{};
        st_in.state = CARVE_STATE_RUNNING;
        st_in.steps_total = e->tick_carve_steps;
        const size_t n_o = order.size(), nb_max = std::max<size_t>(n_o / 2, 1);
        b_n.resize(nb_max);
        b_off.resize(nb_max);
        mem.resize(std::max<size_t>(n_o, 1));
        if (n_o) HIPCHK(hipMemcpyAsync(e->d_order.p, order.data(), n_o * 4, hipMemcpyHostToDevice, e->stream));
        if (stream_now) {
          if (e->stream_seq == 0 || e->stream_seq >= 127) {
            HIPCHK(hipMemsetAsync(e->d_stream_sq.p, 0, size_t(PM_STREAM_SQ) * 8, e->stream));
            HIPCHK(hipMemsetAsync(e->d_stream_row_lo.p, 0, size_t(PM_STREAM_RQ) * 64 * 8, e->stream));
            HIPCHK(hipMemsetAsync(e->d_stream_row_hi.p, 0, size_t(PM_STREAM_RQ) * 64 * 8, e->stream));
            e->stream_seq = 0;
          }
          e->stream_seq += 1;
          a.stream_tag0 = e->stream_seq << 25;
          const uint32_t wgs_want = e->stream_wgs_env ? e->stream_wgs_env : uint32_t(n_o) / 64u + 48u;
          const uint32_t wgs = std::max(1u, std::min(wgs_want, e->n_cus > 8u ? e->n_cus - 4u : 4u));
          HIPCHK(launch_carve_args_put(a, e->d_carve_args.p, e->stream));
          launch_merge_place(e->d_carve_args.p, uint32_t(n_o), 0u, 0u, e->tick_carve_steps, e->stream);
          HIPCHK(launch_carve_stream(e->d_carve_args.p, 0u, wgs, e->stream));
          e->tick_carve_launches += 2;
        } else {
          HIPCHK(hipMemcpyAsync(e->d_status.p, &st_in, sizeof(st_in), hipMemcpyHostToDevice, e->stream));
          HIPCHK(launch_carve_args_put(a, e->d_carve_args.p, e->stream));
          HIPCHK(launch_carve(e->d_carve_args.p, CARVE_F_INIT | CARVE_F_RUN | CARVE_F_ALL, 0, lds, e->stream));
        }
        HIPCHK(hipMemcpyAsync(&st, e->d_status.p, sizeof(st), hipMemcpyDeviceToHost, e->stream));
        HIPCHK(hipMemcpyAsync(b_n.data(), e->d_m_n.p, nb_max * 4, hipMemcpyDeviceToHost, e->stream));
        HIPCHK(hipMemcpyAsync(b_off.data(), e->d_m_off.p, nb_max * 4, hipMemcpyDeviceToHost, e->stream));
        HIPCHK(hipMemcpyAsync(mem.data(), e->d_m_members.p, mem.size() * 4, hipMemcpyDeviceToHost, e->stream));
        HIPCHK(hipStreamSynchronize(e->stream));
        e->tick_carve_launches++;
        if (st.state == CARVE_STATE_OVERFLOW) return set_error(PM_ENOMEM, "merge: batch arrays overflow");
        const bool stream_gave_up = stream_now && st.state == CARVE_STATE_ABORTED;
        if (stream_gave_up) e->tick_stream_aborts++;
        if (stream_now) e->merge_streamed++;
        if (st.state != CARVE_STATE_DONE && st.state != CARVE_STATE_UNCERTAIN && !stream_gave_up)
          return set_error(PM_ENODEV, "merge kernel did not complete");
        const uint32_t nb = st.n_groups;
        if (nb > nb_max || st.n_members > mem.size()) return set_error(PM_ENODEV, "merge: more batches than candidates");
        for (uint32_t k = 0; k < nb; ++k) {
          batches.emplace_back(mem.begin() + b_off[k], mem.begin() + b_off[k] + b_n[k]);
          mark_used(batches.back());
        }
        e->tick_carve_steps = st.steps_total;
        drop_used();
        if (st.state == CARVE_STATE_DONE) break;
        if (stream_gave_up) continue;
        if (order.size() < c.min_group_size) break;
        std::vector<uint32_t> b;
        host_merge_select(e, order, c, &b);
        e->tick_host_resolved++;
        e->tick_carve_steps++;
        if (b.size() < 2) break;
        mark_used(b);
        batches.push_back(std::move(b));
        drop_used();
        if (order.size() < c.min_group_size) break;
      }
      for (uint32_t w : rem) used[w] = 0;
    }

    for (const auto& b : batches) {
      if (b.size() < 2) break;
      if (!e->cfg.switching_enabled) break;
      bool blocked = false;
      if (!e->cfg.prefer_larger_groups)
        for (uint32_t w : b)
          if (e->groups[e->h_group_of[w]].task != PM_NONE) blocked = true;
      if (blocked) break;
      Group gr;
      gr.id = splitmix64_next(&e->id_rng);
      gr.cfg = cfg;
      gr.members = b;
      gr.task = PM_NONE;
      gr.task_uid = 0;
      rc = pick_task_for_config(e, cfg, gr.id, &gr.task);
      if (rc) return rc;
      if (gr.task != PM_NONE) gr.task_uid = e->tasks_have_uid ? e->h_tuid[gr.task] : task_position(e, gr.task);
      for (uint32_t w : b) log_group_event(e, PM_GROUP_DESTROYED, e->groups[e->h_group_of[w]]);
      log_group_event(e, PM_GROUP_CREATED, gr);
      const int32_t slot_new = int32_t(e->groups.size());
      for (uint32_t w : b) {
        e->groups[e->h_group_of[w]].dead = true;
        e->n_dead_groups++;
        e->h_group_of[w] = slot_new;
      }
      e->groups.push_back(std::move(gr));
      e->groups_dirty = true, e->groups_delta_ok = false;
      ++merged;
    }
  }
  compact_groups(e);
  if (n_merged) *n_merged = merged;
  return PM_OK;
}
```

protocol_amd/csrc/pm_engine_state.inc:

```
struct pm_engine {
  pm_engine_config cfg{};
  hipStream_t stream = nullptr;
  hipStream_t stream_owned = nullptr;
  bool own_stream = true;
  hipEvent_t ev[6]{};
  hipEvent_t kev[6]{};
  hipEvent_t k_carve_begin = nullptr;
  hipEvent_t k_compat_end = nullptr;
  bool one_event_behind_carve = false;
  float k_ms_compat = 0, k_ms_carve = 0, k_ms_sweep = 0;
  bool k_sweep_recorded = false, k_compat_recorded = false;
  std::chrono::steady_clock::time_point tick_t0{};
  bool end_event_queued = false;
  uint64_t tick_cand_sum = 0;
  unsigned long long carve_prof[64]{};
  unsigned long long carve_why[25]{};
  uint32_t debug_mem_above = 0;
  uint32_t debug_abort_after = 0;
  uint32_t delta_pushes = 0;
  uint32_t merge_streamed = 0;
  uint32_t merge_stream_min = 512;
  uint32_t prune_mode = 1;
  uint32_t prune_factor = 512;
  uint32_t walk_cap_div = 0;
#ifdef PM_BATCH_LOG
  std::vector<uint32_t> blog;
#endif
  std::mutex mu;

  std::vector<pm_config_row> cfgs;
  std::vector<pm_gpu_alt_row> alts;
  std::vector<uint32_t> model_bits;
  uint32_t model_rows = 0, model_classes = 0;
  bool cls_check_dirty = true;
  uint64_t enabled = ~0ull;
  DevBuf<pm_config_row> d_cfgs;
  DevBuf<pm_gpu_alt_row> d_alts;
  DevBuf<uint32_t> d_model_bits;
  bool have_cfgs = false;

  uint32_t W = 0;
  bool have_workers = false;
  std::vector<uint32_t> h_flags, h_gpu_count, h_gpu_mem, h_gpu_cls, h_cpu_cores, h_ram, h_storage, h_price,
      h_addr_rank;
  std::vector<double> h_lat, h_lon;
  std::vector<uint32_t> h_site;
  DevBuf<uint32_t> d_site, d_c_site, d_cc_site, d_seed_prefix, d_seed_slots, d_prep_block_counts, d_prep_counts;
  DevBuf<uint64_t> d_prop, d_seed_map;
  uint32_t tick_fast_steps = 0;
  DevBuf<uint32_t> d_flags, d_gpu_count, d_gpu_mem, d_gpu_cls, d_cpu_cores, d_ram, d_storage, d_addr_rank;
  DevBuf<double> d_lat, d_lon, d_coslat, d_ux, d_uy, d_uz;
  DevBuf<uint64_t> d_compat;
  bool compat_dirty = true;
  std::vector<uint64_t> h_compat;
  bool h_compat_valid = false;
  bool any_price = false, price_dirty = true;
  std::vector<uint32_t> price_perm;
  SiteMap site_map;
  std::vector<uint32_t> site_pop;
  bool site_bits_dirty = false;
  DevBuf<unsigned char> d_row_stage;
  unsigned char* h_row_pin = nullptr;
  size_t h_row_pin_cap = 0;
  hipEvent_t ev_row_stage = nullptr;

  uint32_t T = 0;
  uint32_t t_cap = 0, t_lo = 0, t_dead = 0;
  uint32_t t_regrowths = 0, t_compactions = 0;
  bool have_tasks = false;
  std::vector<uint64_t> h_tmask, h_tuid, h_tlive;
  std::vector<int64_t> h_created;
  std::vector<uint32_t> h_tprefix;
  bool h_tprefix_valid = false;
  bool tasks_have_uid = false;
  std::unordered_map<uint64_t, uint32_t> uid_to_u;
  bool uid_map_valid = false;
  uint32_t cfg_app_count[PM_MAX_CONFIGS]{};
  bool cfg_app_valid = false;
  DevBuf<uint64_t> d_tmask, d_tplanes, d_tlive;
  DevBuf<int64_t> d_created;
  DevBuf<uint32_t> d_tprefix, d_first_c, d_count_c, d_tdel;
  bool tplanes_dirty = true, tprefix_dirty = true;

  std::vector<Group> groups;
  size_t n_dead_groups = 0;
  bool flags_dirty = false;
  std::vector<int32_t> h_group_of;
  uint64_t id_rng = 0;
  bool groups_dirty = true;
  bool groups_delta_ok = false;
  std::vector<uint32_t> delta_free;
  uint32_t delta_tail_from = PM_NONE;
  bool flags_delta_ok = false;
  std::vector<uint32_t> delta_flags;
  uint32_t* h_delta_pin[2] = {nullptr, nullptr};
  size_t h_delta_cap[2] = {0, 0};
  DevBuf<uint32_t> d_delta[2];
  DevBuf<int32_t> d_group_of;
  DevBuf<uint32_t> d_g_cfg, d_g_n, d_g_off, d_g_task, d_g_task_next, d_members, d_by_rank, d_rank_in_group;
  DevBuf<uint64_t> d_g_id;
  uint32_t d_n_groups = 0, d_n_members = 0;

  DevBuf<uint32_t> d_order;
  uint32_t form_rounds_hint = 0;
  bool tick_needs_merge = false;
  bool events_on = false;
  std::vector<pm_group_event> ev_log;
  std::vector<uint32_t> ev_members;
  DevBuf<double> d_c_lat, d_c_lon, d_c_cos, d_cc_lat, d_cc_lon, d_cc_cos, d_c_u[3], d_cc_u[3];
  DevBuf<uint64_t> d_c_compat, d_keys, d_bits;
  DevBuf<uint32_t> d_slot_pos, d_slot_wid;
  DevBuf<CarveStatus> d_status;
  DevBuf<CarveArgs> d_carve_args;
  DevBuf<BatchDesc> d_desc;
  DevBuf<uint64_t> d_snap;
  DevBuf<uint32_t> d_cell_cnt, d_cell_start, d_pos_cell, d_pos_rank, d_cs_of_pos, d_cs_slot, d_cs_site;
  DevBuf<double> d_cs_u[3];
  DevBuf<double> d_c_pack, d_cs_pack;
  DevBuf<uint64_t> d_cfgbits, d_stream_sq, d_stream_row_lo, d_stream_row_hi, d_stream_trace;
  DevBuf<uint32_t> d_stream_ctl;
  uint32_t stream_seq = 0;
  uint32_t stream_wgs_env = 0;
  uint32_t stream_la_env = 0;
  uint32_t stream_la_div_env = 0;
  uint32_t stream_row_spins_env = 0;
  uint32_t n_cus = 256;
  uint32_t tick_stream_timeouts = 0, tick_stream_tickets = 0, tick_stream_aborts = 0;
  DevBuf<uint64_t> d_ikeys, d_umask;
  DevBuf<uint32_t> d_ivals;
  DevBuf<uint32_t> d_m_cfg, d_m_n, d_m_off, d_m_members;

  DevBuf<uint64_t> d_sel, d_wplanes, d_sel_perm;
  DevBuf<uint32_t> d_first, d_count, d_rank, d_chosen, d_perm;
  DevBuf<pm_assignment> d_table;
  DevBuf<uint32_t> d_task_col;
  const pm_assignment* h_table = nullptr;
  uint64_t groups_epoch = 0, pub_groups_epoch = ~0ull;
  std::unordered_map<uint64_t, uint32_t> slot_of_id;
  uint64_t slot_of_id_epoch = ~0ull;
  uint32_t* h_gstage = nullptr;
  size_t h_gstage_cap = 0;
  const uint32_t *ab_cfg_p = nullptr, *ab_n_p = nullptr, *ab_off_p = nullptr, *ab_mem_p = nullptr;
  CarveStatus* h_status = nullptr;
  hipEvent_t ev_groups = nullptr;
  bool absorb_pending = false;
  uint32_t ab_g0 = 0, ab_g1 = 0, ab_m0 = 0, ab_m1 = 0, ab_solo = 0;
  uint32_t* h_gtask_pinned = nullptr;
  size_t h_gtask_cap = 0;
  pm_assignment* claim_h_table = nullptr;
  uint32_t* claim_h_gtask = nullptr;
  DevBuf<uint32_t> d_nb_idx;
  DevBuf<long long> d_nb_val;

  PubTable pub[2];
  std::atomic<int> pub_cur{-1};
  std::vector<uint64_t*> pub_retired;
  pm_stats last_stats{};

  DevBuf<uint32_t> d_rep_rows, d_rep_why, d_rep_flags, d_rep_live, d_rep_g, d_rep_tprefix, d_rep_cnt, d_rep_task;
  DevBuf<int32_t> d_rep_gof;
  DevBuf<uint32_t> d_spr_idx;
  DevBuf<pm_group_spread_row> d_spr_rows;
  DevBuf<SpreadCfgAcc> d_spr_acc;
  DevBuf<pm_near_query> d_near_q;
  DevBuf<double> d_near_out;
  std::vector<double> h_near_out;

  uint32_t dist_rank = 0, dist_world = 1;
  std::vector<uint8_t> h_shard;
  std::vector<uint32_t> h_own_rows;
  uint32_t dist_cap_t = 0;
  DevBuf<uint8_t> d_shard;
  DevBuf<uint32_t> d_own_rows, d_xrow;
  DevBuf<uint64_t> d_sel_own;
  DevBuf<pm_assignment> d_table_x;
  pm::FormRun* form = nullptr;
  int dist_phase = 0;
  uint32_t dist_n_formed = 0, dist_n_merged = 0;
  uint32_t tick_host_resolved = 0, tick_carve_launches = 0, tick_carve_steps = 0;
  uint32_t tick_props = 0;
  uint64_t tick_prop_keys = 0;
  float k_ms_propose = 0;
  std::vector<hipEvent_t> prop_ev;
  size_t prop_ev_used = 0;
};
```

protocol_amd/csrc/pm_propose.inc:

```
struct NearRow {
  uint64_t key;
  uint64_t tau;
  uint64_t tau_hi;
  uint64_t m1, m2;
  uint32_t s1;
  NEAR_ROW_PROF_FIELDS
};
__device__ __forceinline__ uint64_t wave_shr1_u64(uint64_t v) {
  const uint32_t lo = (uint32_t)__builtin_amdgcn_update_dpp(0, (int)(uint32_t)v, 0x138, 0xF, 0xF, false);
  const uint32_t hi = (uint32_t)__builtin_amdgcn_update_dpp(0, (int)(uint32_t)(v >> 32), 0x138, 0xF, 0xF, false);
  return ((uint64_t)hi << 32) | lo;
}
__device__ __forceinline__ uint64_t near_window(uint64_t tau, uint32_t SB, uint64_t ulps) {
  if (tau >= ((PM_KEY_NOLOC >> SB) << SB)) return tau;
  const uint64_t hi = tau + ulps, floor_bits = 0x03B8F2B061AEA073ull;
  return (hi > floor_bits ? hi : floor_bits) | ((1ull << SB) - 1ull);
}
__device__ __forceinline__ void near_track(NearRow& r, uint64_t k, uint32_t site, bool cand) {
  uint64_t chg = __ballot(cand && (k < r.m1 || (site != r.s1 && k < r.m2)));
  NR_T0;
  NR_CNT(r.p_trk_n, (uint32_t)__popcll(chg));
  while (chg) {
    const uint32_t l = (uint32_t)__builtin_ctzll(chg);
    chg &= chg - 1ull;
// ... 68 lines not shown
__device__ __forceinline__ LaneNet lane_net(uint32_t lane, uint64_t* pack) {
  return LaneNet{lane, (lane ^ 32u) << 2, (63u - lane) << 2, pack};
}
template <uint32_t S, uint32_t KK, uint32_t J>
__device__ __forceinline__ void net_exchange(uint64_t (&w)[S], const LaneNet& ln) {
  const bool want_min = ((ln.lane & J) == 0u) == ((ln.lane & KK) == 0u);
  uint64_t pv[S];
  bool keep[S];
#pragma unroll
  for (uint32_t s = 0; s < S; ++s)
    pv[s] = ((uint64_t)lane_xor_u32<J>((uint32_t)(w[s] >> 32), ln.a_x32) << 32) | lane_xor_u32<J>((uint32_t)w[s], ln.a_x32);
#pragma unroll
  for (uint32_t s = 0; s < S; ++s) keep[s] = (w[s] < pv[s]) == want_min;
#pragma unroll
  for (uint32_t s = 0; s < S; ++s) w[s] = keep[s] ? w[s] : pv[s];
}
template <uint32_t S, uint32_t KK>
__device__ __forceinline__ void net_merge_pass(uint64_t (&w)[S], const LaneNet& ln) {
  if constexpr (KK >= 64u) net_exchange<S, KK, 32u>(w, ln);
  if constexpr (KK >= 32u) net_exchange<S, KK, 16u>(w, ln);
  if constexpr (KK >= 16u) net_exchange<S, KK, 8u>(w, ln);
  if constexpr (KK >= 8u) net_exchange<S, KK, 4u>(w, ln);
  if constexpr (KK >= 4u) net_exchange<S, KK, 2u>(w, ln);
  net_exchange<S, KK, 1u>(w, ln);
}
template <uint32_t S>
__device__ __forceinline__ void net_sort(uint64_t (&w)[S], const LaneNet& ln) {
  net_merge_pass<S, 2u>(w, ln);
  net_merge_pass<S, 4u>(w, ln);
  net_merge_pass<S, 8u>(w, ln);
  net_merge_pass<S, 16u>(w, ln);
  net_merge_pass<S, 32u>(w, ln);
  net_merge_pass<S, 64u>(w, ln);
}
__device__ __forceinline__ uint64_t net_lower(uint64_t a, uint64_t b, const LaneNet& ln) {
  const uint64_t rb = ((uint64_t)(uint32_t)__builtin_amdgcn_ds_bpermute((int)ln.a_rev, (int)(uint32_t)(b >> 32)) << 32) |
                      (uint32_t)__builtin_amdgcn_ds_bpermute((int)ln.a_rev, (int)(uint32_t)b);
  uint64_t m[1] = {a < rb ? a : rb};
  net_merge_pass<1u, 64u>(m, ln);
  return m[0];
}
__device__ __forceinline__ NearRow near_row_bulk4_body(NearRow r, uint64_t k0, uint64_t k1, uint64_t k2, uint64_t k3, uint32_t s0, uint32_t s1,
                                                     uint32_t s2, uint32_t s3, const uint32_t* cc_site_, uint32_t SB, uint64_t ulps,
                                                     uint32_t lane, uint64_t* pack) {
  constexpr uint32_t S = 4u;
  const LaneNet ln = lane_net(lane, pack);
  const auto cc_site = G(cc_site_);
  const uint64_t k[S] = {k0, k1, k2, k3};
  const uint32_t site[S] = {s0, s1, s2, s3};
  NR_CNT(r.p_strides, S);
  NR_SEG0(sg_t);
  uint64_t ent[S];
  uint32_t n_ent = 0u;
#pragma unroll
  for (uint32_t s = 0; s < S; ++s) {
    ent[s] = __ballot(k[s] < r.tau);
    n_ent += (uint32_t)__popcll(ent[s]);
  }
  if (n_ent) {
    NR_T0;
    NR_CNT(r.p_ins_n, n_ent);
    uint64_t low;
    const uint64_t old0 = r.key;
    if (n_ent <= NET_SERIAL_MAX) {
#pragma unroll
      for (uint32_t s = 0; s < S; ++s) {
        uint64_t m = ent[s];
        while (m) {
          const uint32_t l = (uint32_t)__builtin_ctzll(m);
          m &= m - 1ull;
          const uint64_t kk = readlane_u64(k[s], l);
          const uint64_t prev = wave_shr1_u64(r.key);
          const bool gt = r.key > kk, pgt = prev > kk;
          r.key = gt ? (pgt ? prev : kk) : r.key;
        }
      }
      low = 0ull;
    } else if (n_ent <= NET_PACK_KEYS) {
      uint32_t base = 0u;
#pragma unroll
      for (uint32_t s = 0; s < S; ++s) {
        if (k[s] < r.tau) ln.pack[base + __builtin_amdgcn_mbcnt_hi((uint32_t)(ent[s] >> 32), __builtin_amdgcn_mbcnt_lo((uint32_t)ent[s], 0u))] = k[s];
        base += (uint32_t)__popcll(ent[s]);
      }
      __builtin_amdgcn_fence(__ATOMIC_SEQ_CST, "wavefront");
      NR_SEG(r, 0, sg_t);
      if (n_ent <= 64u) {
        uint64_t one[1] = {ln.lane < n_ent ? ln.pack[ln.lane] : ~0ull};
        __builtin_amdgcn_fence(__ATOMIC_SEQ_CST, "wavefront");
        net_sort<1u>(one, ln);
        low = one[0];
      } else {
        uint64_t two[2] = {ln.pack[ln.lane], 64u + ln.lane < n_ent ? ln.pack[64u + ln.lane] : ~0ull};
        __builtin_amdgcn_fence(__ATOMIC_SEQ_CST, "wavefront");
        net_sort<2u>(two, ln);
        low = net_lower(two[0], two[1], ln);
      }
    } else {
      uint64_t w[S];
#pragma unroll
      for (uint32_t s = 0; s < S; ++s) w[s] = k[s];
      net_sort<S>(w, ln);
      const uint64_t r1 = ((uint64_t)(uint32_t)__builtin_amdgcn_ds_bpermute((int)ln.a_rev, (int)(uint32_t)(w[1] >> 32)) << 32) |
                          (uint32_t)__builtin_amdgcn_ds_bpermute((int)ln.a_rev, (int)(uint32_t)w[1]);
      const uint64_t r3 = ((uint64_t)(uint32_t)__builtin_amdgcn_ds_bpermute((int)ln.a_rev, (int)(uint32_t)(w[3] >> 32)) << 32) |
                          (uint32_t)__builtin_amdgcn_ds_bpermute((int)ln.a_rev, (int)(uint32_t)w[3]);
      uint64_t m[2] = {w[0] < r1 ? w[0] : r1, w[2] < r3 ? w[2] : r3};
      net_merge_pass<2u, 64u>(m, ln);
      low = net_lower(m[0], m[1], ln);
    }
    const uint64_t old = old0;
    if (n_ent > NET_SERIAL_MAX) r.key = net_lower(old, low, ln);
    NR_ADD(r.p_ins_t);
    NR_SEG(r, 1, sg_t);
    r.tau = readlane_u64(r.key, 63u);
    r.tau_hi = near_window(r.tau, SB, ulps);
    const bool ev = old > r.tau && old < r.tau_hi;
    if (__ballot(ev)) {
      NR_CNT(r.p_ev_n, 1u);
      const uint32_t es = ev ? cc_site[(uint32_t)(old & ((1ull << SB) - 1ull))] : 0u;
      near_track(r, old, es, ev);
    }
    NR_SEG(r, 2, sg_t);
  }
#pragma unroll
  for (uint32_t s = 0; s < S; ++s) {
    const bool nm = k[s] > r.tau && k[s] < r.tau_hi;
    if (__ballot(nm)) near_track(r, k[s], site[s], nm);
  }
  NR_SEG(r, 3, sg_t);
  return r;
}
__device__ __noinline__ NearRow near_row_bulk4(NearRow r, uint64_t k0, uint64_t k1, uint64_t k2, uint64_t k3, uint32_t s0, uint32_t s1,
                                               uint32_t s2, uint32_t s3, const uint32_t* cc_site_, uint32_t SB, uint64_t ulps,
                                               uint32_t lane, uint64_t* pack) {
  return near_row_bulk4_body(r, k0, k1, k2, k3, s0, s1, s2, s3, cc_site_, SB, ulps, lane, pack);
}
template <uint32_t S, bool INLINE = false>
__device__ __forceinline__ void near_row_offer_bulk(NearRow& r, const uint64_t (&k)[S], const uint32_t (&site)[S], const uint32_t* cc_site,
                                                    uint32_t SB, uint64_t ulps, const LaneNet& ln) {
  static_assert(S == 4u, "four strides a call");
  uint64_t any_hi = 0ull;
#pragma unroll
  for (uint32_t s = 0; s < S; ++s) any_hi |= __ballot(k[s] < r.tau_hi);
  if (!any_hi) {
    NR_CNT(r.p_strides, S);
    return;
  }
  NR_SEG0(call_t);
  if constexpr (INLINE) r = near_row_bulk4_body(r, k[0], k[1], k[2], k[3], site[0], site[1], site[2], site[3], cc_site, SB, ulps, ln.lane, ln.pack);
  else r = near_row_bulk4(r, k[0], k[1], k[2], k[3], site[0], site[1], site[2], site[3], cc_site, SB, ulps, ln.lane, ln.pack);
  NR_SEG(r, 5, call_t);
  NR_CNT(r.p_seg[4], 1u);
}

#ifndef PROP_TILE
#define PROP_TILE 512u
#endif
#define PROP_TILE_PER_THREAD (PROP_TILE / 256u)
#define PROP_TILE_WORDS (PROP_TILE / 64u)
struct TileBuf {
  double x[PROP_TILE], y[PROP_TILE], z[PROP_TILE];
  uint32_t site[PROP_TILE];
  uint64_t alive[PROP_TILE_WORDS], loc[PROP_TILE_WORDS];
};
struct TileRegs {
  double x[PROP_TILE_PER_THREAD], y[PROP_TILE_PER_THREAD], z[PROP_TILE_PER_THREAD];
  uint32_t site[PROP_TILE_PER_THREAD];
  uint64_t bm;
};
template <typename BP>
__device__ __forceinline__ void tile_fetch(const CarveArgs& p, BP alive, BP loc, uint32_t lw, uint32_t n_list,
                                           uint32_t tile, uint32_t tid, TileRegs& r) {
#pragma unroll
  for (uint32_t h = 0; h < PROP_TILE_PER_THREAD; ++h) {
    const uint32_t t = tile * PROP_TILE + h * 256u + tid;
    const uint32_t tc = t < n_list ? t : n_list - 1u;
    r.x[h] = G(p.cc_ux)[tc];
    r.y[h] = G(p.cc_uy)[tc];
    r.z[h] = G(p.cc_uz)[tc];
    r.site[h] = G(p.cc_site)[tc];
  }
  const uint32_t j = tile * PROP_TILE_WORDS + (tid % PROP_TILE_WORDS);
  r.bm = (tid < 2u * PROP_TILE_WORDS && j < lw) ? (tid < PROP_TILE_WORDS ? alive[j] : loc[j]) : 0ull;
}
__device__ __forceinline__ void tile_store(TileBuf& tb, uint32_t tid, const TileRegs& r) {
#pragma unroll
  for (uint32_t h = 0; h < PROP_TILE_PER_THREAD; ++h) {
    const uint32_t o = h * 256u + tid;
    tb.x[o] = r.x[h];
    tb.y[o] = r.y[h];
    tb.z[o] = r.z[h];
    tb.site[o] = r.site[h];
  }
  if (tid < PROP_TILE_WORDS) tb.alive[tid] = r.bm;
  else if (tid < 2u * PROP_TILE_WORDS) tb.loc[tid - PROP_TILE_WORDS] = r.bm;
}
__device__ __forceinline__ void tile_keys(const CarveArgs& p, const TileBuf& tb, uint32_t tile, uint32_t lane, uint32_t s,
                                          bool shared, uint32_t ssite, const SeedGeo& sg, uint32_t SB, uint64_t ulps,
                                          NearRow& q, uint32_t& n_mine) {
  const bool form = UNI(p.mode) != CARVE_MODE_MERGE;
#pragma unroll 1
  for (uint32_t h = 0; h < PROP_TILE / 256u; ++h) {
    double x[4], y[4], z[4];
    uint32_t si[4];
    uint64_t aw[4], lwd[4];
#pragma unroll
    for (uint32_t v = 0; v < 4u; ++v) {
      const uint32_t u = h * 4u + v, o = u * 64u + lane;
      aw[v] = tb.alive[u];
      lwd[v] = tb.loc[u];
      x[v] = tb.x[o];
      y[v] = tb.y[o];
      z[v] = tb.z[o];
      si[v] = tb.site[o];
    }
#pragma unroll
    for (uint32_t v = 0; v < 4u; ++v) {
      const uint32_t u = h * 4u + v, t = tile * PROP_TILE + u * 64u + lane;
      const bool located = (lwd[v] >> lane) & 1ull;
      const bool counts = ((aw[v] >> lane) & 1ull) && t != s && !(located && t < s && (form || (shared && si[v] == ssite)));
      const double dx = x[v] - sg.ux, dy = y[v] - sg.uy, dz = z[v] - sg.uz;
      double a = 0.25 * fma(dx, dx, fma(dy, dy, dz * dz));
      const bool same_site = located && si[v] == ssite;
      const bool near = counts && located && a < PM_A_CHORD_MIN && !same_site;
      a = same_site ? 0.0 : a;
      if (__ballot(near)) {
        if (near) a = hav_a(sg.lat, sg.lon, sg.cos, G(p.cc_lat)[t], G(p.cc_lon)[t], G(p.cc_cos)[t]);
      }
      const uint64_t kl = pack_key(located ? (uint64_t)__double_as_longlong(a) : PM_KEY_NOLOC, t, SB);
      near_row_offer(q, counts ? kl : ~0ull, si[v], G(p.cc_site), SB, ulps);
      n_mine += counts ? 1u : 0u;
    }
  }
}

__device__ __forceinline__ uint32_t cell_g_for(uint32_t n) {
  return n >= PM_CELL_BIG_N ? PM_CELL_G_MAX : n >= PM_CELL_MIN_N ? PM_CELL_G_MAX / 2u : 0u;
}
__device__ __forceinline__ uint32_t cell_coord(double v, uint32_t g) {
  const double t = fmax((v + 1.0) * (double)(g >> 1), 0.0);
  const uint32_t c = (uint32_t)t;
  return c < g ? c : g - 1u;
}
__device__ __forceinline__ uint64_t cell_bound_key(double gx, double gy, double gz, uint32_t SB) {
  gx = fmax(gx - 1e-9, 0.0);
  gy = fmax(gy - 1e-9, 0.0);
  gz = fmax(gz - 1e-9, 0.0);
  const double a = 0.25 * (gx * gx + gy * gy + gz * gz) * (1.0 - 1e-6);
  return pack_key((uint64_t)__double_as_longlong(a), 0u, SB);
}
__device__ __forceinline__ uint64_t candidate_key(const CarveArgs& p, const SeedGeo& sg, uint32_t ssite, double x, double y, double z,
                                                  uint32_t si, uint32_t t, bool located, bool counts, uint32_t SB, NearRow& q) {
  const double dx = x - sg.ux, dy = y - sg.uy, dz = z - sg.uz;
  double a = 0.25 * fma(dx, dx, fma(dy, dy, dz * dz));
  const bool same_site = located && si == ssite;
  const bool near = counts && located && a < PM_A_CHORD_MIN && !same_site;
  a = same_site ? 0.0 : a;
  if (__ballot(near)) {
    NR_T0;
    NR_CNT(q.p_hav_n, 1u);
    if (near) a = hav_a(sg.lat, sg.lon, sg.cos, G(p.cc_lat)[t], G(p.cc_lon)[t], G(p.cc_cos)[t]);
    NR_ADD(q.p_hav_t);
  }
  const uint64_t kl = pack_key(located ? (uint64_t)__double_as_longlong(a) : PM_KEY_NOLOC, t, SB);
  return counts ? kl : ~0ull;
}
__device__ __forceinline__ void offer_candidate(const CarveArgs& p, const SeedGeo& sg, uint32_t ssite, double x, double y,
                                                double z, uint32_t si, uint32_t t, bool located, bool counts, uint32_t SB,
                                                uint64_t ulps, NearRow& q, uint32_t& n_mine) {
  const uint64_t kl = candidate_key(p, sg, ssite, x, y, z, si, t, located, counts, SB, q);
  near_row_offer(q, kl, si, G(p.cc_site), SB, ulps);
  n_mine += counts ? 1u : 0u;
}
#define CELL_BUF 768u
#ifndef STREAM_BULK_UPTO
#define STREAM_BULK_UPTO 0x40000000u
#endif
struct BulkCtx {
  uint32_t seen;
  LaneNet ln;
  BULK_REC_FIELDS
};
template <bool STREAM = false>
__device__ __forceinline__ void cell_drain(const CarveArgs& p, uint32_t* wl, uint32_t& nb, uint32_t lane, uint32_t s, bool shared,
                                           uint32_t ssite, const SeedGeo& sg, uint32_t SB, uint64_t ulps, NearRow& q,
                                           uint32_t& n_mine, BulkCtx* bulk = nullptr) {
  const auto cs_site = G((const uint32_t*)p.cs_site);
  const auto cs_x = G((const double*)p.cs_ux);
  const auto cs_y = G((const double*)p.cs_uy);
  const auto cs_z = G((const double*)p.cs_uz);
  const double* const pack = p.cs_pack;
  __builtin_amdgcn_fence(__ATOMIC_SEQ_CST, "wavefront");
  constexpr uint32_t NV = STREAM ? 4u : 2u;
  for (uint32_t k0 = 0; k0 < nb; k0 += NV * 64u) {
    uint32_t t[NV], si[NV];
    double x[NV], y[NV], z[NV];
    bool in[NV];
#pragma unroll
    for (uint32_t v = 0; v < NV; ++v) {
      const uint32_t k = k0 + v * 64u + lane;
      in[v] = k < nb;
      const uint32_t kc = in[v] ? k : 0u;
      const uint32_t ic = wl[kc];
      t[v] = wl[CELL_BUF + kc];
      if (STREAM) {
// ... 513 lines not shown
```

protocol_amd/csrc/pm_stream.inc:

```

enum { SLW_TREQ = PM_STREAM_TP,
       SLW_PAY,
       SLW_TISSUED,
       SLW_SCANW, SLW_SCANLO, SLW_SCANHI,
       SLW_TIMEOUTS,
       SLW_LA,
       SLW_TEND,
       SLW_ACKT, SLW_ACKP0, SLW_ACKP1, SLW_ACKP2, SLW_ACKP3, SLW_ACKP4,
       SLW_NCAND,
       SLW_P_CI, SLW_P_CI1, SLW_P_PAY, SLW_P_PAY1, SLW_P_MAX, SLW_P_MAX1, SLW_P_T0, SLW_P_T01, SLW_P_CNT, SLW_P_CNT1,
       SLW_P_SCANW, SLW_P_SCANW1, SLW_P_SCANLO, SLW_P_SCANLO1, SLW_P_SCANHI, SLW_P_SCANHI1,
       SLW_WORDS };
static_assert(SLW_TREQ == PM_STREAM_SLW_TREQ && SLW_PAY == PM_STREAM_SLW_PAY, "the words carve_fast_steps reads");
static_assert(SLW_WORDS <= PM_STREAM_TP + 32u, "ticket state fits its LDS region");
#ifndef STREAM_NPARK
#define STREAM_NPARK 5u
#endif
#ifndef STREAM_PARK_NB
#define STREAM_PARK_NB 16u
#endif
#ifndef STREAM_NAP_TICKETER
#define STREAM_NAP_TICKETER 4
#endif
#ifndef STREAM_NAP_PARK
// ... 1563 lines not shown
      stream_park<BIG>(p, c, l_alive, l_stage, sl_words, wave == 1 ? 0u : wave < 5u ? 4u : wave - 4u);
    }
    lds_barrier();
    const uint32_t act = red.f_action;
    c.n_cand = red.f_n_cand;
    c.total_available = red.f_total_available;
    c.n_groups = red.f_n_groups;
    c.mem_off = red.f_mem_off;
    c.steps = red.f_steps;
    c.fast_steps = red.f_fast;
    c.cand_sum = red.f_cand_sum;
    seed_cur = red._spare1;
    lds_barrier();
    if (act == FAST_TINY) continue;
    if (act == FAST_TAIL && merge) {
      for (;;) {
        const int rc = exact_step();
        if (rc != STEP_CONTINUE) return rc;
      }
    }
    if (act == FAST_TAIL) {
      const int ta = stream_first_come(p, red, c, l_alive, l_stage);
      if (tid == 0) STREAM_TRACE(12, (uint32_t)ta, c.steps);
      if (ta == FAST_DONE) return STEP_BREAK;
      if (ta == FAST_OVERFLOW) return STEP_OVERFLOW;
      return stream_tail_serial<BIG>(p, red, c, l_site, l_alive, l_loc, steps_before);
    }
    if (act == FAST_DONE) return STEP_BREAK;
    if (act == FAST_OVERFLOW) return STEP_OVERFLOW;
    if (act == FAST_ABORT) return STEP_ABORT;
    if (act == FAST_REPROPOSE) {
      if (tid == 0) {
        typedef __attribute__((address_space(3))) uint32_t sl_u32;
        sl_u32* const SL = (sl_u32*)sl_words;
        SL[SLW_PAY] = (SL[SLW_PAY] & 0x00FC0000u) | ((uint32_t)SROW_BITMAP << 24);
        p.status->stream_switches += 1u;
      }
      c.n_start = 0u;
      __syncthreads();
      continue;
    }
    if (act == FAST_RANOUT && c.steps - refresh_at >= 8u) {
      if (tid == 0) {
        typedef __attribute__((address_space(3))) uint32_t sl_u32;
        sl_u32* const SL = (sl_u32*)sl_words;
        SL[SLW_SCANW] = 0u;
        SL[SLW_SCANLO] = SL[SLW_SCANHI] = 0xFFFFFFFFu;
        SL[SLW_TEND] = PM_NONE;
        SL[SLW_TREQ] = SL[SLW_TISSUED];
        SL[SLW_NCAND] = c.n_cand;
        p.status->stream_refreshes += 1u;
        __hip_atomic_store(&p.stream_ctl[SC_DROP], STREAM_DROP_WORD((SL[SLW_PAY] >> 18) & 63u, SL[SLW_TISSUED]), __ATOMIC_RELAXED,
                           __HIP_MEMORY_SCOPE_AGENT);
      }
      seed_cur = PM_NONE;
      refresh_at = c.steps;
      __syncthreads();
      continue;
    }
    const int rc = exact_step();
    if (rc != STEP_CONTINUE) return rc;
    if (merge && c.steps - refresh_at >= 8u) {
      if (tid == 0) {
        typedef __attribute__((address_space(3))) uint32_t sl_u32;
        sl_u32* const SL = (sl_u32*)sl_words;
        SL[SLW_SCANW] = 0u;
        SL[SLW_SCANLO] = SL[SLW_SCANHI] = 0xFFFFFFFFu;
        SL[SLW_TEND] = PM_NONE;
        SL[SLW_TREQ] = SL[SLW_TISSUED];
        SL[SLW_NCAND] = c.n_cand;
        p.status->stream_refreshes += 1u;
        __hip_atomic_store(&p.stream_ctl[SC_DROP], STREAM_DROP_WORD((SL[SLW_PAY] >> 18) & 63u, SL[SLW_TISSUED]), __ATOMIC_RELAXED,
                           __HIP_MEMORY_SCOPE_AGENT);
      }
      seed_cur = PM_NONE;
      refresh_at = c.steps;
      __syncthreads();
    }
  }
}

#define STREAM_WL_WORDS 4608u
__device__ __forceinline__ bool stream_drain(const CarveArgs& p, const uint32_t* wl, uint32_t nb, uint32_t lane, uint32_t s, bool shared,
                                             uint32_t ssite, const SeedGeo& sg, uint32_t SB, uint64_t ulps, NearRow& q, uint32_t& n_mine,
                                             BulkCtx& bulk, uint32_t ci, uint32_t ticket) {
  const double* const pack = p.c_pack;
  const bool located_only = UNI(p.mode) == CARVE_MODE_MERGE;
  const bool form = !located_only;
  struct Batch {
    uint32_t t[4];
    pm_d4 rec[4];
  };
  auto fetch = [&](Batch& bt, uint32_t k0) {
#pragma unroll
    for (uint32_t v = 0; v < 4u; ++v) {
      const uint32_t k = k0 + v * 64u + lane;
      const uint32_t tc = wl[k < nb ? k : 0u];
      bt.t[v] = k < nb ? tc : 0xFFFFFFFFu;
      bt.rec[v] = pack_load(pack, PM_ROWB(4u) ? lane : tc);
    }
  };
  auto eval = [&](const Batch& bt, uint32_t n_in_batch) {
    uint64_t kk[4];
    uint32_t ss[4];
    const uint32_t n_in = n_in_batch;
    PM_PROF(const uint64_t ek0 = PM_TICKS();)
#pragma unroll
    for (uint32_t v = 0; v < 4u; ++v) {
      const bool in = bt.t[v] != 0xFFFFFFFFu;
      const uint32_t tv = in ? bt.t[v] : 0u;
      const bool located = pack_located(bt.rec[v]);
      ss[v] = pack_site(bt.rec[v]);
      const bool counts = in && tv != s && !(located && tv < s && (form || (shared && ss[v] == ssite))) && (located || !located_only);
      kk[v] = PM_ROWB(2u) ? (counts ? (((uint64_t)(tv * 2654435761u) << SB) | tv) : ~0ull)
                          : candidate_key(p, sg, ssite, bt.rec[v].x, bt.rec[v].y, bt.rec[v].z, ss[v], counts ? tv : 0u, located, counts, SB, q);
      n_mine += counts ? 1u : 0u;
    }
    PM_PROF(const uint64_t ek1 = PM_TICKS(); q.p_key_t += ek1 - ek0;)
    PM_REC(if (bulk.rec_keys == 0) bulk.rec_keys = STREAM_CLOCK();)
    if (PM_ROWB(1u)) {
      q.m1 ^= kk[0] ^ kk[1] ^ kk[2] ^ kk[3];
    } else if (UNI(bulk.seen) < STREAM_BULK_UPTO) {
      near_row_offer_bulk<4u, true>(q, kk, ss, p.cc_site, SB, ulps, bulk.ln);
    } else {
#pragma unroll
      for (uint32_t v = 0; v < 4u; ++v) {
        if (v * 64u >= n_in) continue;
        near_row_offer(q, kk[v], ss[v], G(p.cc_site), SB, ulps);
      }
    }
    PM_PROF(q.p_off_t += PM_TICKS() - ek1;)
    bulk.seen += n_in;
  };
  if (nb == 0u) return false;
  if (PM_ROWB(8u)) {
    n_mine += nb / 64u;
    return false;
  }
  const auto drop_w = G(p.stream_ctl) + SC_DROP;
  Batch cur, nxt;
  fetch(cur, 0u);
  for (uint32_t k0 = 0; k0 < nb; k0 += 256u) {
    const bool more = k0 + 256u < nb;
    const uint32_t dropw = ld_ag32(drop_w);
    if (more) fetch(nxt, k0 + 256u);
    DRAIN_PROF_WAIT(more);
    eval(cur, nb - k0 < 256u ? nb - k0 : 256u);
    DRAIN_PROF_BOOK(q);
    if (STREAM_DROPPED(UNI(dropw), ci, ticket)) return true;
    if (more) cur = nxt;
  }
  return false;
}
__device__ __forceinline__ bool stream_bitmap_sweep(const CarveArgs& p, const uint64_t* cfg64, uint32_t n, uint32_t* wl, uint32_t lane,
                                                    uint32_t s, bool shared, uint32_t ssite, const SeedGeo& sg, uint32_t SB,
                                                    uint64_t ulps, NearRow& q, uint32_t& n_mine, BulkCtx& bulk, uint32_t ci, uint32_t ticket) {
  const auto freeg = G((const unsigned long long*)p.bits_scratch);
  const auto cfgb = G(cfg64);
  const uint32_t lw = (n + 63u) >> 6;
  uint32_t nb = 0u;
  SWEEP_PROF_DECL;
  const auto locg = G((const unsigned long long*)p.loc_g);
  const uint32_t sw = UNI(p.mode) != CARVE_MODE_MERGE ? s >> 6 : 0u;
  const unsigned long long s_below = UNI(p.mode) != CARVE_MODE_MERGE ? (1ull << (s & 63u)) - 1ull : 0ull;
  auto word = [&](uint32_t j) -> unsigned long long {
    if (j >= lw) return 0ull;
    unsigned long long a = ld_ag(&freeg[j]) & cfgb[j];
    if (j <= sw) a &= ~(locg[j] & (j < sw ? ~0ull : s_below));
    return a;
  };
  unsigned long long a_n = word(lane);
  for (uint32_t j0 = 0; j0 < lw; j0 += 64u) {
    unsigned long long a = a_n;
    a_n = word(j0 + 64u + lane);
    const uint32_t cw = (uint32_t)__popcll(a);
    const uint32_t incl = wave_incl_scan_u32(cw);
    uint32_t o = nb + incl - cw;
    const uint32_t base = (j0 + lane) * 64u;
    for (; a; a &= a - 1ull) wl[o++] = base + (uint32_t)__builtin_ctzll(a);
    nb += (uint32_t)__builtin_amdgcn_readlane((int)incl, 63);
    PM_REC(if (bulk.rec_pass == 0) bulk.rec_pass = STREAM_CLOCK();)
    SWEEP_PROF_MARK(bp_pass, bp_np, 1u);
    if (nb >= 512u || j0 + 64u >= lw) {
      __builtin_amdgcn_fence(__ATOMIC_SEQ_CST, "wavefront");
      const uint32_t take = j0 + 64u >= lw ? nb : (nb & ~255u);
      if (stream_drain(p, wl, take, lane, s, shared, ssite, sg, SB, ulps, q, n_mine, bulk, ci, ticket)) return true;
      SWEEP_PROF_MARK(bp_drain, bp_nd, (take + 255u) >> 8);
      __builtin_amdgcn_fence(__ATOMIC_SEQ_CST, "wavefront");
      const uint32_t left = nb - take;
      uint32_t mv[4];
#pragma unroll
      for (uint32_t v = 0; v < 4u; ++v) mv[v] = v * 64u + lane < left ? wl[take + v * 64u + lane] : 0u;
      __builtin_amdgcn_fence(__ATOMIC_SEQ_CST, "wavefront");
#pragma unroll
      for (uint32_t v = 0; v < 4u; ++v)
        if (v * 64u + lane < left) wl[v * 64u + lane] = mv[v];
      nb = left;
    }
  }
  SWEEP_PROF_BOOK(q);
  return false;
}

__device__ __forceinline__ void stream_proposer(const CarveArgs& p, unsigned char* s_raw) {
  const uint32_t lane = threadIdx.x & 63u, wave = threadIdx.x >> 6;
  if (wave >= PM_STREAM_PROP_WAVES) return;
  const auto st = G((const CarveStatus*)p.status);
  if (st->state != CARVE_STATE_RUNNING) return;
  const uint32_t n = st->n_eligible;
  if (n == 0u || n > PM_CARVE_BIG_SLOTS) return;
  const uint32_t SB = n > PM_CARVE_SLOTS ? PM_CARVE_SLOT_BITS_BIG : PM_CARVE_SLOT_BITS;
  const double TIE_BAND = n > PM_CARVE_SLOTS ? PM_TIE_BAND_BIG : PM_TIE_BAND;
  const uint64_t WINDOW_ULPS = n > PM_CARVE_SLOTS ? (1ull << 25) : (1ull << 20);
  const uint32_t cell_g = st->cell_g;
  static_assert(STREAM_WL_WORDS >= 2u * CELL_BUF, "the walk's buffer fits the sweep's");
  static_assert(size_t(CARVE_WAVES) * STREAM_WL_WORDS * 4u <= PM_STREAM_LDS_BYTES, "one candidate buffer per wave");
  uint32_t* wl = reinterpret_cast<uint32_t*>(s_raw) + wave * STREAM_WL_WORDS;
  const auto ctl = G(p.stream_ctl);
  const auto sq = G((const unsigned long long*)p.stream_sq);
  const auto row_lo = G(p.stream_row_lo);
  const auto row_hi = G(p.stream_row_hi);
  const uint32_t tag0 = UNI(p.stream_tag0);
  static_assert(size_t(CARVE_WAVES) * STREAM_WL_WORDS * 4u + size_t(CARVE_WAVES) * NET_PACK_KEYS * 8u <= PM_STREAM_LDS_BYTES,
                "a packing list per wave behind the buffers");
  BulkCtx bulk = {0u, lane_net(lane, reinterpret_cast<uint64_t*>(s_raw + size_t(CARVE_WAVES) * STREAM_WL_WORDS * 4u) + wave * NET_PACK_KEYS)};
  for (;;) {
    uint32_t t = 0u;
    if (lane == 0u) t = atomicAdd(&p.stream_ctl[SC_CLAIM], 1u);
    t = UNI(t);
    unsigned long long g;
    uint32_t nap = 8u;
    for (uint32_t spins = 0u;;) {
      g = ld_ag(&sq[t & (PM_STREAM_SQ - 1u)]);
      if (UNI((uint32_t)(g >> 32)) == tag0 + t) break;
      if ((spins & 255u) == 255u && UNI(ld_ag32(&ctl[SC_QUIT]))) return;
      if (nap >= 32u) __builtin_amdgcn_s_sleep(STREAM_NAP_LONG);
      else if (nap >= 16u) __builtin_amdgcn_s_sleep(STREAM_NAP_LONG < 32 ? STREAM_NAP_LONG : 32);
      else __builtin_amdgcn_s_sleep(STREAM_NAP_LONG < 16 ? STREAM_NAP_LONG : 16);
      nap = nap < 32u ? nap << 1 : nap;
      if (++spins > PM_STREAM_IDLE_SPINS) {
        if (lane == 0u) atomicAdd(&p.stream_ctl[SC_GAVE_UP], 1u);
        return;
      }
    }
    if (UNI((uint32_t)g) == 0xFFFFFFFFu) return;
    const uint64_t t_seen = __builtin_amdgcn_s_memtime();
    PM_PROF(const uint64_t bt0 = t_seen;)
    const uint32_t pay = UNI((uint32_t)g);
    const uint32_t s = pay & 0x3FFFFu, mode = (pay >> 24) & 3u, ci = (pay >> 18) & 63u;
    if (s >= n) continue;
    if (STREAM_DROPPED(UNI(ld_ag32(&ctl[SC_DROP])), ci, t)) continue;
    const uint64_t* cfg64 = p.cfgbits + (size_t)ci * p.bits_stride;
    const uint32_t ssite = G(p.cc_site)[s];
    const SeedGeo sg = {G(p.cc_lat)[s], G(p.cc_lon)[s], G(p.cc_cos)[s], G(p.cc_ux)[s], G(p.cc_uy)[s], G(p.cc_uz)[s]};
    const bool shared = (ssite & 0x80000000u) != 0u;
    NearRow q = {~0ull, ~0ull, ~0ull, ~0ull, ~0ull, 0xFFFFFFFFu};
    uint32_t n_mine = 0;
    bulk.seen = 0u;
    PM_REC(bulk.rec_pass = bulk.rec_keys = 0; const uint64_t rec_seen = STREAM_CLOCK();)
    PM_PROF(asm volatile("s_waitcnt vmcnt(0)" ::: "memory"); const uint64_t bt_geo = PM_TICKS();)
    bool sweep = true;
    if (mode == SROW_WALK && cell_g) {
      const uint32_t stop_r = p.prune_mode != 3u ? cell_walk<true>(p, wl, cell_g, PM_CELL_RMAX, lane, s, shared, ssite, sg, SB, WINDOW_ULPS, q, n_mine, (const uint32_t*)cfg64, &bulk) : 0u;
      sweep = !stop_r;
      if (sweep) {
        q = NearRow{~0ull, ~0ull, ~0ull, ~0ull, ~0ull, 0xFFFFFFFFu};
        n_mine = 0;
        bulk.seen = 0u;
        if (lane == 0) atomicAdd(&p.status->prune_fallbacks, 1u);
      }
    } else if (mode == SROW_SWEEP) {
      list_sweep_solo<true>(p, n, lane, s, shared, ssite, sg, SB, WINDOW_ULPS, q, n_mine, cfg64);
      sweep = false;
    }
    if (UNI(sweep) && stream_bitmap_sweep(p, cfg64, n, wl, lane, s, shared, ssite, sg, SB, WINDOW_ULPS, q, n_mine, bulk, ci, t)) {
      if (lane == 0u) atomicAdd(&p.stream_ctl[SC_LET_BE], 1u);
      continue;
    }
    PM_PROF(const uint64_t bt1 = PM_TICKS();)
    PM_REC(const uint64_t rec_swept = STREAM_CLOCK();)
    uint64_t mine;
    const uint32_t meta = near_row_finish(p, q, true, PM_PROP_KMAX, SB, TIE_BAND, lane, &mine);
    PM_REC(const uint64_t rec_fin = STREAM_CLOCK() + (meta & 0u);)
    if (p.count_keys) {
      const uint32_t swept = wave_sum(n_mine);
      if (lane == 0) {
        atomicAdd((unsigned long long*)&p.status->prop_keys, (unsigned long long)swept);
        atomicAdd(&p.status->n_props, 1u);
      }
    }
    static_assert(PM_STREAM_SQ == PM_STREAM_RQ, "the ticket ring tells when a row slot has a newer owner");
    if (__builtin_amdgcn_s_memtime() - t_seen > STREAM_LATE_ROW_TICKS) {
      const unsigned long long g2 = ld_ag(&sq[t & (PM_STREAM_SQ - 1u)]);
      if (UNI((uint32_t)(g2 >> 32)) != tag0 + t) continue;
    }
    const size_t rb = (size_t)(t & (PM_STREAM_RQ - 1u)) * 64u + ((lane + 1u) & 63u);
    const unsigned long long tagw = (unsigned long long)(tag0 + t) << 32;
    st_ag(&row_hi[rb], tagw | (lane == 63u ? 0ull : (unsigned long long)(uint32_t)(mine >> 32)));
    asm volatile("s_waitcnt vmcnt(0)" ::: "memory");
    st_ag(&row_lo[rb], tagw | (lane == 63u ? (unsigned long long)meta : (unsigned long long)(uint32_t)mine));
    PROP_REC_ROW(t, mode, n_mine, rec_seen, bulk, rec_swept, rec_fin);
    PROP_PROF_ROW(t, mode, q, n_mine, bt0, bt_geo, bt1);
  }
}

__global__ __launch_bounds__(CARVE_THREADS) void carve_stream_kernel(const CarveArgs* __restrict__ pa, uint32_t start_ci) {
  const CarveArgs& p = *pa;
  extern __shared__ __attribute__((aligned(16))) unsigned char s_raw[];
  if (blockIdx.x != 0u) {
    stream_proposer(p, s_raw);
    return;
  }
  uint64_t* part = reinterpret_cast<uint64_t*>(s_raw);
  uint64_t* lds_alive = part + CARVE_WAVES * PM_CARVE_PART;
  uint64_t* lds_loc = lds_alive + PM_CARVE_SLOTS / 64;
  uint32_t* lds_wid = reinterpret_cast<uint32_t*>(lds_loc + PM_CARVE_SLOTS / 64);
  uint32_t* lds_site = lds_wid + PM_CARVE_SLOTS;
  uint64_t* lds_key = reinterpret_cast<uint64_t*>(lds_site + PM_CARVE_SLOTS);
  uint32_t* sel_out = reinterpret_cast<uint32_t*>(lds_key + PM_CARVE_SLOTS);
  BlockRed& red = *reinterpret_cast<BlockRed*>(sel_out + PM_CARVE_SEL_CAP);
  uint32_t* sl_words = reinterpret_cast<uint32_t*>(s_raw + PM_CARVE_LDS_BYTES);

  const uint32_t tid = threadIdx.x, lane = tid & 63u, wave = tid >> 6;
  const auto st = G(p.status);
  const auto ctl = G(p.stream_ctl);
  if (st->state != CARVE_STATE_RUNNING) {
    if (tid == 0) st_ag32(&ctl[SC_QUIT], 1u);
    return;
  }
  const uint32_t n = st->n_eligible;
  const uint32_t lw = (n + 63u) >> 6;
  uint32_t exit_state = CARVE_STATE_DONE, stop_ci = p.n_avail;
  StepCtx c;
  c.mode = p.mode;
  c.proximity = p.proximity;
  c.use_props = true;
  c.steps = 0;
  c.fast_steps = 0;
  c.cand_sum = 0;
  c.total_available = st->total_available;
  c.n_groups = st->n_groups;
  c.mem_off = st->n_members;
  c.n_list = n;
  c.n_cand = 0;
  c.min_s = c.max_s = 1;
  c.cfg = 0;
  ctx_set_geometry(c);
  const uint32_t groups_at_entry = c.n_groups;
  const uint32_t steps_before = st->steps_total;
  const bool big = c.big;
  uint64_t* r_alive = big ? reinterpret_cast<uint64_t*>(lds_wid) : lds_alive;
  uint64_t* r_loc = big ? reinterpret_cast<uint64_t*>(lds_site) : lds_loc;
  uint32_t ci = start_ci;
  if (n > PM_CARVE_BIG_SLOTS) {
    exit_state = CARVE_STATE_ABORTED;
    stop_ci = ci;
  } else if (n > 0u) {
    for (uint32_t j = tid; j < lw; j += CARVE_THREADS) r_loc[j] = G(p.loc_g)[j];
    if (!big)
      for (uint32_t sl = tid; sl < n; sl += CARVE_THREADS) lds_site[sl] = G(p.cc_site)[sl];
    for (uint32_t k = tid; k < (uint32_t)SLW_WORDS; k += CARVE_THREADS) sl_words[k] = (k == SLW_P_CI || k == SLW_P_CI1 || k == SLW_TEND) ? PM_NONE : 0u;
    __syncthreads();
    const auto master = G(p.alive_g);
    const auto cfgbits = G((const uint64_t*)p.cfgbits);
    const uint32_t cell_g = st->cell_g, n_indexed = st->n_indexed;
    auto count_candidates = [&](uint32_t cx) -> uint32_t {
      uint32_t cnt = 0;
      for (uint32_t j = tid; j < lw; j += CARVE_THREADS) cnt += (uint32_t)__popcll(master[j] & cfgbits[(size_t)cx * p.bits_stride + j]);
      cnt = wave_sum(cnt);
      __syncthreads();
      if (lane == 0) red.a[wave] = cnt;
      __syncthreads();
      uint32_t tot = 0;
#pragma unroll
      for (uint32_t k = 0; k < CARVE_WAVES; ++k) tot += red.a[k];
      __syncthreads();
      return tot;
    };
    auto row_mode = [&](uint32_t n_cand, uint32_t* switch_at) -> uint32_t {
      *switch_at = 0u;
      if (!cell_g || !p.prune_mode) return SROW_BITMAP;
      if (p.prune_mode >= 2u) return SROW_WALK;
// ... 80 lines not shown
        for (uint32_t cx = ci + 1u; cx < p.n_avail && have < 2u; ++cx) {
          if (c.total_available < p.min_size[cx]) continue;
          const bool slotted = sl_words[SLW_P_CI] == cx || sl_words[SLW_P_CI1] == cx;
          uint32_t nx = 0u;
          if (!slotted) {
            nx = count_candidates(cx);
            if (nx < p.min_size[cx] || nx == 0u) continue;
          }
          ++have;
          if (slotted || !(p.max_size[cx] > 1u && p.max_size[cx] - 1u < PM_PROP_KMAX)) continue;
          if (tid == 0) {
            const uint32_t k = sl_words[SLW_P_CI] == PM_NONE ? 0u : sl_words[SLW_P_CI1] == PM_NONE ? 1u : 2u;
            if (k < 2u) {
              uint32_t sw_next = 0u;
              sl_words[SLW_P_CI + k] = cx;
              sl_words[SLW_P_PAY + k] = (cx << 18) | (row_mode(nx, &sw_next) << 24);
              sl_words[SLW_P_MAX + k] = look_ahead(nx, p.max_size[cx]);
              sl_words[SLW_P_CNT + k] = 0u;
              sl_words[SLW_P_T0 + k] = 0u;
              sl_words[SLW_P_SCANW + k] = 0u;
              sl_words[SLW_P_SCANLO + k] = sl_words[SLW_P_SCANHI + k] = 0xFFFFFFFFu;
            }
          }
          __syncthreads();
        }
      }
      __syncthreads();
      seed_cur0 = red._spare2;
      __syncthreads();
      if (tid == 0) STREAM_TRACE(1, ci, n_cand);
      PROF_MARK(33);
      int rc;
      if (!big)
        rc = stream_run_config<false>(p, red, c, lds_site, lds_key, r_alive, r_loc, part, sel_out,
                                      reinterpret_cast<uint32_t*>(lds_key), sl_words, steps_before, seed_cur0);
      else
        rc = stream_run_config<true>(p, red, c, p.cc_site, p.keys, r_alive, r_loc, part, sel_out,
                                     reinterpret_cast<uint32_t*>(lds_key), sl_words, steps_before, seed_cur0);
      __syncthreads();
      if (tid == 0) st_ag32(&ctl[SC_DROP], STREAM_DROP_WORD(ci, sl_words[SLW_TISSUED]));
      PROF_MARK(34);
      if (rc == STEP_UNCERTAIN || rc == STEP_OVERFLOW || rc == STEP_ABORT) {
        exit_state = rc == STEP_UNCERTAIN ? CARVE_STATE_UNCERTAIN : rc == STEP_ABORT ? CARVE_STATE_ABORTED : CARVE_STATE_OVERFLOW;
        stop_ci = ci;
        break;
      }
      if (tid == 0) acc_done += 1u;
    }
    if (tid == 0) {
      st->why[3] += acc_done;
      st->stream_pre_used += acc_pre_used;
      st->stream_pre_lost += acc_pre_lost;
      st->stream_listed += acc_listed;
      st->pruned_batches += acc_pruned;
    }
  }
  if (tid == 0) {
    st_ag32(&ctl[SC_QUIT], 1u);
    ctl[SC_FINISH] = 1u;
  }
  if (n > 0u && n <= PM_CARVE_BIG_SLOTS) {
    const uint32_t q_lo = sl_words[SLW_TISSUED];
    const uint32_t q_hi = ld_ag32(&ctl[SC_CLAIM]) + (gridDim.x - 1u) * PM_STREAM_PROP_WAVES + 64u;
    const auto sq = G(p.stream_sq);
    const uint32_t tag0 = p.stream_tag0;
    for (uint32_t t = q_lo + tid; t < q_hi && t - q_lo < PM_STREAM_SQ; t += CARVE_THREADS)
      st_ag(&sq[t & (PM_STREAM_SQ - 1u)], ((unsigned long long)(tag0 + t) << 32) | 0xFFFFFFFFull);
  }
  __syncthreads();
  if (tid == 0) {
    st->state = exit_state;
    st->n_groups = c.n_groups;
    st->n_members = c.mem_off;
    st->steps_total = steps_before + c.steps;
    st->stop_ci = stop_ci;
    st->cand_sum += c.cand_sum;
    st->cur_ci = exit_state == CARVE_STATE_DONE ? p.n_avail : ci;
    st->n_list = n;
    st->total_available = c.total_available;
    st->g_lo = groups_at_entry;
    st->g_hi = c.n_groups;
    st->fast_steps += c.fast_steps;
    st->slow_steps += c.steps - c.fast_steps;
    st->n_batches += 1u;
    if (n > 0u && n <= PM_CARVE_BIG_SLOTS) {
      st->stream_timeouts += sl_words[SLW_TIMEOUTS];
      st->stream_tickets += sl_words[SLW_TISSUED];
    }
  }
}

__global__ __launch_bounds__(256) void carve_finish_kernel(const CarveArgs* __restrict__ pa) {
  const CarveArgs& p = *pa;
  const auto st = G(p.status);
  const auto ctl = G(p.stream_ctl);
  __shared__ uint32_t s_last;
  if (ctl[SC_FINISH]) {
    const uint32_t g_lo = st->g_lo, g_hi = st->g_hi;
    const uint32_t total = gridDim.x * 256u;
    const uint32_t id_g0 = p.id_g0, m0 = p.stage_m0, cap_g = p.stage_cap_g, cap_m = p.stage_cap_m;
    const bool stage = p.stage_cfg != nullptr;
    uint32_t solo = 0;
    for (uint32_t g = g_lo + blockIdx.x * 256u + threadIdx.x; g < g_hi; g += total) {
      const uint32_t off = G(p.g_off)[g], gn = G(p.g_n)[g];
      const uint32_t k = g - id_g0;
      for (uint32_t j = 0; j < gn; ++j) {
        const uint32_t w = G(p.order)[G(p.members)[off + j]];
        G(p.members)[off + j] = w;
        if (p.mode == CARVE_MODE_FORM) G(p.group_of)[w] = (int32_t)g;
        if (stage && off + j - m0 < cap_m) p.stage_mem[off + j - m0] = w;
      }
      if (p.g_id_out) {
        unsigned long long z = p.id_state + (unsigned long long)(k + 1u) * 0x9E3779B97F4A7C15ull;
        z = (z ^ (z >> 30)) * 0xBF58476D1CE4E5B9ull;
        z = (z ^ (z >> 27)) * 0x94D049BB133111EBull;
        p.g_id_out[g] = z ^ (z >> 31);
        p.g_task_out[g] = PM_NONE;
      }
      if (stage && k < cap_g) {
        p.stage_cfg[k] = G(p.g_cfg)[g];
        p.stage_n[k] = gn;
        p.stage_off[k] = off;
      }
      solo += gn == 1u ? 1u : 0u;
    }
    solo = wave_sum(solo);
    if ((threadIdx.x & 63u) == 0u && solo) atomicAdd(&p.status->n_solo, solo);
  }
  if (!p.h_status) return;
  __syncthreads();
  if (threadIdx.x == 0) {
    __threadfence();
    s_last = atomicAdd(&p.stream_ctl[SC_FINISH_TICKET], 1u);
  }
  __syncthreads();
  if (s_last != gridDim.x - 1u) return;
  const auto src = G((const uint32_t*)p.status);
  uint32_t* dst = (uint32_t*)p.h_status;
  for (uint32_t k = threadIdx.x; k < (uint32_t)(sizeof(CarveStatus) / 4u); k += 256u) dst[k] = ld_ag32((const stream_gu32*)(src + k));
}

hipError_t launch_carve_stream(const CarveArgs* d_args, uint32_t start_ci, uint32_t n_prop_wgs, hipStream_t s) {
  hipLaunchKernelGGL(carve_stream_kernel, dim3(1u + n_prop_wgs), dim3(CARVE_THREADS), PM_STREAM_LDS_BYTES, s, d_args, start_ci);
  hipLaunchKernelGGL(carve_finish_kernel, dim3(128), dim3(256), 0, s, d_args);
  return hipGetLastError();
}

#ifdef PM_ROW_BENCH
__global__ __launch_bounds__(CARVE_THREADS) void carve_row_bench_kernel(const CarveArgs* __restrict__ pa, uint32_t s, uint32_t ci, uint32_t reps,
                                                                        unsigned long long* __restrict__ out) {
  const CarveArgs& p = *pa;
  extern __shared__ __attribute__((aligned(16))) unsigned char s_raw[];
  const uint32_t lane = threadIdx.x & 63u, wave = threadIdx.x >> 6;
  if (wave != 0u) return;
  const auto st = G((const CarveStatus*)p.status);
  const uint32_t n = st->n_eligible;
  if (n == 0u || n > PM_CARVE_BIG_SLOTS || s >= n) return;
  const uint32_t SB = n > PM_CARVE_SLOTS ? PM_CARVE_SLOT_BITS_BIG : PM_CARVE_SLOT_BITS;
  const double TIE_BAND = n > PM_CARVE_SLOTS ? PM_TIE_BAND_BIG : PM_TIE_BAND;
  const uint64_t WINDOW_ULPS = n > PM_CARVE_SLOTS ? (1ull << 25) : (1ull << 20);
  uint32_t* wl = reinterpret_cast<uint32_t*>(s_raw);
  BulkCtx bulk = {0u, lane_net(lane, reinterpret_cast<uint64_t*>(s_raw + size_t(CARVE_WAVES) * STREAM_WL_WORDS * 4u))};
  const uint64_t* cfg64 = p.cfgbits + (size_t)ci * p.bits_stride;
  unsigned long long t_all = 0, t_geo = 0, t_sweep = 0, t_fin = 0, check = 0;
  uint32_t swept = 0;
  for (uint32_t rep = 0; rep < reps; ++rep) {
    const uint64_t t0 = __builtin_amdgcn_s_memtime();
    const uint32_t ssite = G(p.cc_site)[s];
    const SeedGeo sg = {G(p.cc_lat)[s], G(p.cc_lon)[s], G(p.cc_cos)[s], G(p.cc_ux)[s], G(p.cc_uy)[s], G(p.cc_uz)[s]};
    const bool shared = (ssite & 0x80000000u) != 0u;
    NearRow q = {~0ull, ~0ull, ~0ull, ~0ull, ~0ull, 0xFFFFFFFFu};
    uint32_t n_mine = 0;
    bulk.seen = 0u;
    asm volatile("s_waitcnt vmcnt(0)" ::: "memory");
    const uint64_t t1 = __builtin_amdgcn_s_memtime();
    (void)stream_bitmap_sweep(p, cfg64, n, wl, lane, s, shared, ssite, sg, SB, WINDOW_ULPS, q, n_mine, bulk, ci, 0x01FFFFF0u);
    const uint64_t t2 = __builtin_amdgcn_s_memtime();
    uint64_t mine = q.m1;
    const uint32_t meta = PM_ROWB(1u) ? 0u : near_row_finish(p, q, true, PM_PROP_KMAX, SB, TIE_BAND, lane, &mine);
    const uint64_t t3 = __builtin_amdgcn_s_memtime() + (meta & 0u);
    t_all += t3 - t0;
    t_geo += t1 - t0;
    t_sweep += t2 - t1;
    t_fin += t3 - t2;
    swept = wave_sum(n_mine);
    check = mine * (lane + 1u) + meta;
  }
  unsigned long long cs = check;
  for (uint32_t o = 32u; o; o >>= 1) cs += __shfl_xor(cs, o, 64);
  if (lane == 0u) {
    out[0] = t_all;
    out[1] = reps;
    out[2] = swept;
    out[3] = cs;
    out[4] = t_geo;
    out[5] = t_sweep;
    out[6] = t_fin;
  }
}
#endif
```

protocol_amd/engine.py:

```python
from __future__ import annotations

import ctypes as C
import os

import numpy as np

from . import build as _build

PM_NONE = 0xFFFFFFFF
PM_MAX_CONFIGS = 64
PM_OK, PM_EINVAL, PM_ENODEV, PM_ENOMEM, PM_ESTATE, PM_ERANGE, PM_EPARSE, PM_EPANIC = 0, -1, -2, -3, -4, -5, -6, -7
CHOOSE_FIRST, CHOOSE_SEEDED = 0, 1

(W_HAS_SPECS, W_HAS_GPU, W_GPU_COUNT, W_GPU_MEM, W_GPU_MODEL, W_HAS_CPU, W_CPU_CORES, W_RAM, W_STORAGE,
 W_HEALTHY, W_HAS_P2P, W_HAS_LOC) = (1 << i for i in range(12))
R_HAS_REQ, R_CPU, R_CPU_CORES, R_RAM, R_STORAGE = (1 << i for i in range(5))
G_COUNT, G_MODEL, G_MEM, G_MEM_MIN, G_MEM_MAX, G_TOT_MIN, G_TOT_MAX = (1 << i for i in range(7))

config_row_dt = np.dtype([("flags", "<u4"), ("cpu_cores", "<u4"), ("ram_mb", "<u4"), ("storage_gb", "<u4"),
                          ("alt_begin", "<u4"), ("alt_count", "<u4"), ("min_group_size", "<u4"),
                          ("max_group_size", "<u4")], align=True)
alt_row_dt = np.dtype([("flags", "<u4"), ("count", "<u4"), ("memory_mb", "<u4"), ("memory_mb_min", "<u4"),
                       ("memory_mb_max", "<u4"), ("total_memory_min", "<u4"), ("total_memory_max", "<u4"),
                       ("model_row", "<u4")], align=True)
# ... 495 lines not shown
    def newest_task(self) -> int:
        t = C.c_uint32(0)
        check(lib().pm_newest_task(self._h, C.byref(t)))
        return t.value

    def tick(self) -> dict:
        s = Stats()
        check(lib().pm_tick(self._h, C.byref(s)))
        return s.as_dict()

    def last_stats(self) -> dict:
        s = Stats()
        check(lib().pm_last_stats(self._h, C.byref(s)))
        return s.as_dict()

    def device_task_column(self):
        p, n = C.c_uint64(0), C.c_uint32(0)
        check(lib().pm_device_task_column(self._h, C.byref(p), C.byref(n)))
        return p.value, n.value

    def set_stream(self, hip_stream: int | None):
        check(lib().pm_set_stream(self._h, C.c_void_p(hip_stream or 0)))

    def dist_configure(self, rank: int, world: int, shard_of_worker=None):
        sh = None if shard_of_worker is None else _arr(shard_of_worker, np.uint8)
        if sh is not None:
            assert len(sh) == self.W
        check(lib().pm_dist_configure(self._h, rank, world, sh.ctypes.data if sh is not None and len(sh) else None))

    def dist_tick_begin(self):
        check(lib().pm_dist_tick_begin(self._h))

    def dist_carve_wait(self):
        check(lib().pm_dist_carve_wait(self._h))

    def dist_match_begin(self) -> DistXfer:
        x = DistXfer()
        check(lib().pm_dist_match_begin(self._h, C.byref(x)))
        return x

    def dist_tick_end(self) -> dict:
        s = Stats()
        check(lib().pm_dist_tick_end(self._h, C.byref(s)))
        return s.as_dict()

    def match_per_task_device(self):
        b, c, n = C.c_uint64(0), C.c_uint64(0), C.c_uint32(0)
        check(lib().pm_match_per_task_device(self._h, C.byref(b), C.byref(c), C.byref(n)))
        return b.value, c.value, n.value

    def hbm_triad_gbs(self, n_doubles: int = 1 << 27, reps: int = 5) -> float:
        L = lib()
        L.pm_debug_hbm_triad.argtypes = [C.c_void_p, C.c_uint64, C.c_uint32, C.POINTER(C.c_double)]
        L.pm_debug_hbm_triad.restype = C.c_int32
        out = C.c_double(0)
        check(L.pm_debug_hbm_triad(self._h, n_doubles, reps, C.byref(out)))
        return out.value

    def debug_mem_lists_above(self, n: int):
        L = lib()
        L.pm_debug_mem_lists_above.argtypes = [C.c_void_p, C.c_uint32]
        L.pm_debug_mem_lists_above.restype = C.c_int32
        check(L.pm_debug_mem_lists_above(self._h, n))

    def debug_stream_abort_after(self, n: int):
        L = lib()
        L.pm_debug_stream_abort_after.argtypes = [C.c_void_p, C.c_uint32]
        L.pm_debug_stream_abort_after.restype = C.c_int32
        check(L.pm_debug_stream_abort_after(self._h, n))

    def debug_merge_streamed(self) -> int:
        L = lib()
        L.pm_debug_merge_streamed.argtypes = [C.c_void_p, C.POINTER(C.c_uint32)]
        L.pm_debug_merge_streamed.restype = C.c_int32
        n = C.c_uint32(0)
        check(L.pm_debug_merge_streamed(self._h, C.byref(n)))
        return n.value

    def debug_delta_pushes(self) -> int:
        L = lib()
        L.pm_debug_delta_pushes.argtypes = [C.c_void_p, C.POINTER(C.c_uint32)]
        L.pm_debug_delta_pushes.restype = C.c_int32
        n = C.c_uint32(0)
        check(L.pm_debug_delta_pushes(self._h, C.byref(n)))
        return n.value

    def debug_task_space(self) -> dict:
        L = lib()
        L.pm_debug_carve_prof.argtypes = [C.c_void_p, C.POINTER(C.c_ulonglong), C.c_uint32]
        L.pm_debug_carve_prof.restype = C.c_int32
        out = (C.c_ulonglong * 97)()
        check(L.pm_debug_carve_prof(self._h, out, 97))
        keys = ("t_lo", "t_cap", "T", "t_dead", "regrowths", "compactions", "n_groups", "n_dead_groups", "retired_buffers")
        return dict(zip(keys, (int(v) for v in out[88:97])))

    def debug_row_networks(self, keys, sites, n_per_wave: int, slot_bits: int, ulps: int, upto: int):
        import numpy as np
        L = lib()
        keys = np.ascontiguousarray(keys, dtype=np.uint64)
        sites = np.ascontiguousarray(sites, dtype=np.uint32)
        assert keys.size % n_per_wave == 0 and sites.size == 1 << slot_bits
        n_waves = keys.size // n_per_wave
        rows = np.zeros((n_waves, 64), dtype=np.uint64)
        mism = (C.c_uint32 * 2)()
        L.pm_debug_row_networks.argtypes = [C.c_void_p, C.c_void_p, C.c_void_p, C.c_uint32, C.c_uint32, C.c_uint32, C.c_uint64,
                                            C.c_uint32, C.c_void_p, C.POINTER(C.c_uint32)]
        L.pm_debug_row_networks.restype = C.c_int32
        check(L.pm_debug_row_networks(self._h, keys.ctypes.data, sites.ctypes.data, n_waves, n_per_wave, slot_bits, ulps, upto,
                                      rows.ctypes.data, mism))
        return int(mism[0]), int(mism[1]), rows

    def debug_distance_keys(self, lat1, lon1, lat2, lon2, slots=None):
        import numpy as np
        L = lib()
        n = len(lat1)
        if slots is None:
            slots = np.zeros(n)
        inp = np.concatenate([np.asarray(lat1, np.float64), np.asarray(lat2, np.float64), np.asarray(lon1, np.float64),
                              np.asarray(lon2, np.float64), np.asarray(slots, np.float64)])
        assert inp.size == 5 * n
        out = np.zeros((n, 20), dtype=np.float64)
        L.pm_debug_distance_keys.argtypes = [C.c_void_p, C.c_void_p, C.c_uint32, C.c_uint32, C.c_void_p]
        L.pm_debug_distance_keys.restype = C.c_int32
        check(L.pm_debug_distance_keys(self._h, inp.ctypes.data, n, 0, out.ctypes.data))
        bits = out.view(np.uint64)
        return {"sin_dlat": out[:, 0].copy(), "sin_dlon": out[:, 1].copy(), "cos1": out[:, 2].copy(), "u1": out[:, 3:6].copy(),
                "cos2": out[:, 6].copy(), "u2": out[:, 7:10].copy(), "hav_a": out[:, 10].copy(), "prox_a": out[:, 11].copy(),
                "chord": out[:, 12] == 1.0, "candidate_key": out[:, 13].copy(), "packed_prox": bits[:, 14:17].copy(),
                "packed_hav": bits[:, 17:20].copy()}

    def debug_sin_band(self, x):
        import numpy as np
        L = lib()
        x = np.ascontiguousarray(x, dtype=np.float64)
        out = np.zeros(x.size, dtype=np.float64)
        L.pm_debug_distance_keys.argtypes = [C.c_void_p, C.c_void_p, C.c_uint32, C.c_uint32, C.c_void_p]
        L.pm_debug_distance_keys.restype = C.c_int32
        check(L.pm_debug_distance_keys(self._h, x.ctypes.data, x.size, 1, out.ctypes.data))
        return out

    def debug_key_geometry(self) -> dict:
        L = lib()
        out = (C.c_double * 8)()
        L.pm_debug_distance_keys.argtypes = [C.c_void_p, C.c_void_p, C.c_uint32, C.c_uint32, C.c_void_p]
        L.pm_debug_distance_keys.restype = C.c_int32
        check(L.pm_debug_distance_keys(self._h, None, 0, 2, out))
        return {"chord_min": out[0], "a_max_safe": out[1], "bands": (out[2], out[3], out[4]),
                "slot_bits": (int(out[5]), int(out[6]), int(out[7]))}

    def debug_carve_counters(self) -> dict:
        L = lib()
        L.pm_debug_carve_prof.argtypes = [C.c_void_p, C.POINTER(C.c_ulonglong), C.c_uint32]
        L.pm_debug_carve_prof.restype = C.c_int32
        out = (C.c_ulonglong * 98)()
        check(L.pm_debug_carve_prof(self._h, out, 98))
        w = [int(v) for v in out[32:56]]
        return {"why": w[:8], "batches": w[8], "void_launches": w[9], "pruned_batches": w[10], "prune_fallbacks": w[11],
                "cell_g": w[12], "n_indexed": w[13],
                "stream": w[14], "stream_tickets": w[15], "stream_timeouts": w[16], "stream_switches": w[17],
                "stream_listed": w[18], "stream_wgs": w[19], "stream_aborts": w[20], "slow_steps": w[21],
                "stream_pre_used": w[22], "stream_pre_lost": w[23], "stream_refreshes": int(out[97])}

    def debug_prune_mode(self, mode: int):
        L = lib()
        L.pm_debug_prune_mode.argtypes = [C.c_void_p, C.c_uint32]
        L.pm_debug_prune_mode.restype = C.c_int32
        check(L.pm_debug_prune_mode(self._h, mode))

    def lookup(self, worker: int) -> Assignment:
        a = Assignment()
        check(lib().pm_lookup_task_for_worker(self._h, worker, C.byref(a)))
        return a
```

Before: 1112 billion.

## Split one streamed proposal row across four waves of a workgroup

Adds a shared-row proposer mode, on by default, in which the four proposer waves of a workgroup cooperatively sweep one ticket's candidate bitmap. Each wave takes every fourth word; three waves post partial top-k results to LDS and wave 0 merges and delivers the row. Mode 2 falls back to per-wave rows when the candidate count for a config is below a threshold. The stream kernel's default workgroup count is doubled to compensate. This cuts per-row latency for long sweeps at the cost of workgroup barriers, LDS merge work and less row-level parallelism.

Measured after the change: 1114 billion, median of 2. Within noise of the previous version (+0.2%).

```diff
diff --git a/protocol_amd/csrc/pm_device.h b/protocol_amd/csrc/pm_device.h
--- a/protocol_amd/csrc/pm_device.h
+++ b/protocol_amd/csrc/pm_device.h
@@ -199,7 +199,7 @@
   uint32_t stream_pre_used;
   uint32_t stream_pre_lost;
   uint32_t stream_refreshes;
-  uint32_t _pad_sr;
+  uint32_t stream_shared_rows;
   uint32_t cell_g;
   uint32_t n_indexed;
   uint32_t pruned_batches;
@@ -282,6 +282,7 @@
   uint32_t stream_la, stream_row_spins;
   uint32_t stream_la_div;
   uint32_t debug_abort_after;
+  uint32_t stream_shared, _pad_ss;
   unsigned long long id_state;
   uint32_t id_g0, stage_m0;
   uint32_t stage_cap_g, stage_cap_m;
diff --git a/protocol_amd/csrc/pm_engine.cpp b/protocol_amd/csrc/pm_engine.cpp
--- a/protocol_amd/csrc/pm_engine.cpp
+++ b/protocol_amd/csrc/pm_engine.cpp
@@ -109,6 +109,9 @@
   if (const char* v = getenv("PM_STREAM_ROW_SPINS")) {
     const long f = atol(v);
     if (f > 0 && f < (1l << 24)) e->stream_row_spins_env = uint32_t(f);
+  }
+  if (const char* v = getenv("PM_STREAM_SHARED_ROWS")) {
+    if (v[0] >= '0' && v[0] <= '2' && !v[1]) e->stream_shared_env = uint32_t(v[0] - '0');
   }
   if (const char* v = getenv("PM_STREAM_LA_DIV")) {
     const long f = atol(v);
diff --git a/protocol_amd/csrc/pm_engine_carve.inc b/protocol_amd/csrc/pm_engine_carve.inc
--- a/protocol_amd/csrc/pm_engine_carve.inc
+++ b/protocol_amd/csrc/pm_engine_carve.inc
@@ -226,6 +226,7 @@
     a->stream_la = e->stream_la_env;
     a->stream_la_div = e->stream_la_div_env;
     a->stream_row_spins = e->stream_row_spins_env;
+    a->stream_shared = e->stream_shared_env;
     a->debug_abort_after = e->debug_abort_after;
   }
   return PM_OK;
@@ -441,7 +442,7 @@
   int32_t rc = fill_carve_args(e, &a, CARVE_MODE_FORM, 0, r->stream);
   if (rc) return rc;
   if (r->stream) {
-    uint32_t wgs = e->stream_wgs_env ? e->stream_wgs_env : r->n_elig_hint / 64u + 48u;
+    uint32_t wgs = e->stream_wgs_env ? e->stream_wgs_env : (r->n_elig_hint / 64u + 48u) * (e->stream_shared_env ? 2u : 1u);
     const uint32_t max_wgs = e->n_cus > 8u ? e->n_cus - 4u : 4u;
     r->stream_wgs = std::max(1u, std::min(wgs, max_wgs));
     a.stream_tag0 = ((e->stream_seq == 0 || e->stream_seq >= 127) ? 1u : e->stream_seq + 1u) << 25;
@@ -589,6 +590,7 @@
   e->carve_why[22] = st.stream_pre_used;
   e->carve_why[23] = st.stream_pre_lost;
   e->carve_why[24] = st.stream_refreshes;
+  e->carve_why[25] = st.stream_shared_rows;
 #ifdef PM_BATCH_LOG
   e->blog.assign(st.blog, st.blog + 3 * std::min<uint32_t>(st.blog_n, 512u));
 #endif
diff --git a/protocol_amd/csrc/pm_engine_debug.inc b/protocol_amd/csrc/pm_engine_debug.inc
--- a/protocol_amd/csrc/pm_engine_debug.inc
+++ b/protocol_amd/csrc/pm_engine_debug.inc
@@ -9,6 +9,7 @@
                                      e->groups.size(), e->n_dead_groups, e->pub_retired.size()};
   for (uint32_t k = 88; k < cap && k < 97; ++k) out[k] = inc[k - 88];
   if (cap > 97u) out[97] = e->carve_why[24];
+  if (cap > 98u) out[98] = e->carve_why[25];
   return PM_OK;
 }
 
@@ -226,18 +227,18 @@
   unsigned long long *d_ones = nullptr, *d_out = nullptr;
   CarveArgs* d_h = nullptr;
   int32_t rc = PM_OK;
-  if (hipMalloc((void**)&d_ones, h.bits_stride * 8) != hipSuccess || hipMalloc((void**)&d_out, 64) != hipSuccess ||
+  if (hipMalloc((void**)&d_ones, h.bits_stride * 8) != hipSuccess || hipMalloc((void**)&d_out, 128) != hipSuccess ||
       hipMalloc((void**)&d_h, sizeof(h)) != hipSuccess) {
     rc = set_error(PM_ENOMEM, "row bench buffers");
   } else {
     (void)hipMemset(d_ones, 0xFF, h.bits_stride * 8);
-    (void)hipMemset(d_out, 0, 64);
+    (void)hipMemset(d_out, 0, 128);
     h.bits_scratch = (uint64_t*)d_ones;
     (void)hipMemcpy(d_h, &h, sizeof(h), hipMemcpyHostToDevice);
     if (launch_row_bench(d_h, seed, ci, reps, mode, d_out, e->stream) != hipSuccess || hipStreamSynchronize(e->stream) != hipSuccess)
       rc = set_error(PM_ENODEV, "row bench");
     else
-      (void)hipMemcpy(out, d_out, 64, hipMemcpyDeviceToHost);
+      (void)hipMemcpy(out, d_out, 128, hipMemcpyDeviceToHost);
     out[7] = seed;
   }
   if (d_ones) (void)hipFree(d_ones);
diff --git a/protocol_amd/csrc/pm_engine_merge.inc b/protocol_amd/csrc/pm_engine_merge.inc
--- a/protocol_amd/csrc/pm_engine_merge.inc
+++ b/protocol_amd/csrc/pm_engine_merge.inc
@@ -139,7 +139,7 @@
           }
           e->stream_seq += 1;
           a.stream_tag0 = e->stream_seq << 25;
-          const uint32_t wgs_want = e->stream_wgs_env ? e->stream_wgs_env : uint32_t(n_o) / 64u + 48u;
+          const uint32_t wgs_want = e->stream_wgs_env ? e->stream_wgs_env : (uint32_t(n_o) / 64u + 48u) * (e->stream_shared_env ? 2u : 1u);
           const uint32_t wgs = std::max(1u, std::min(wgs_want, e->n_cus > 8u ? e->n_cus - 4u : 4u));
           HIPCHK(launch_carve_args_put(a, e->d_carve_args.p, e->stream));
           launch_merge_place(e->d_carve_args.p, uint32_t(n_o), 0u, 0u, e->tick_carve_steps, e->stream);
diff --git a/protocol_amd/csrc/pm_engine_state.inc b/protocol_amd/csrc/pm_engine_state.inc
--- a/protocol_amd/csrc/pm_engine_state.inc
+++ b/protocol_amd/csrc/pm_engine_state.inc
@@ -14,7 +14,7 @@
   bool end_event_queued = false;
   uint64_t tick_cand_sum = 0;
   unsigned long long carve_prof[64]{};
-  unsigned long long carve_why[25]{};
+  unsigned long long carve_why[26]{};
   uint32_t debug_mem_above = 0;
   uint32_t debug_abort_after = 0;
   uint32_t delta_pushes = 0;
@@ -124,6 +124,7 @@
   uint32_t stream_la_env = 0;
   uint32_t stream_la_div_env = 0;
   uint32_t stream_row_spins_env = 0;
+  uint32_t stream_shared_env = 2;
   uint32_t n_cus = 256;
   uint32_t tick_stream_timeouts = 0, tick_stream_tickets = 0, tick_stream_aborts = 0;
   DevBuf<uint64_t> d_ikeys, d_umask;
diff --git a/protocol_amd/csrc/pm_propose.inc b/protocol_amd/csrc/pm_propose.inc
--- a/protocol_amd/csrc/pm_propose.inc
+++ b/protocol_amd/csrc/pm_propose.inc
@@ -244,6 +244,37 @@
   else r = near_row_bulk4(r, k[0], k[1], k[2], k[3], site[0], site[1], site[2], site[3], cc_site, SB, ulps, ln.lane, ln.pack);
   NR_SEG(r, 5, call_t);
   NR_CNT(r.p_seg[4], 1u);
+}
+
+#define NEAR_PART_U64 68u
+__device__ __forceinline__ void near_part_post(uint64_t* part, const NearRow& q, uint32_t n_evaluated, uint32_t lane) {
+  part[lane] = q.key;
+  if (lane == 0u) {
+    part[64] = q.m1;
+    part[65] = q.m2;
+    part[66] = (uint64_t)q.s1 | ((uint64_t)n_evaluated << 32);
+  }
+}
+__device__ __forceinline__ uint32_t near_row_merge_parts(NearRow& q, const uint64_t* parts, const uint32_t* cc_site_, uint32_t SB,
+                                                         uint64_t ulps, const LaneNet& ln) {
+  const auto cc_site = G(cc_site_);
+  const uint64_t smask = (1ull << SB) - 1ull;
+  const uint32_t lane = ln.lane;
+  uint64_t kk[4];
+  uint32_t ss[4];
+#pragma unroll
+  for (uint32_t v = 0; v < 3u; ++v) kk[v] = parts[v * NEAR_PART_U64 + lane];
+  kk[3] = ~0ull;
+  ss[3] = 0u;
+#pragma unroll
+  for (uint32_t v = 0; v < 3u; ++v) ss[v] = kk[v] != ~0ull ? cc_site[(uint32_t)(kk[v] & smask)] : 0u;
+  const uint32_t pv = lane < 3u ? lane : lane < 6u ? lane - 3u : 0u;
+  const uint64_t tk = lane < 6u ? parts[pv * NEAR_PART_U64 + 64u + (lane < 3u ? 0u : 1u)] : ~0ull;
+  const uint64_t sw = parts[pv * NEAR_PART_U64 + 66u];
+  const uint32_t ts = lane < 3u ? (uint32_t)sw : tk != ~0ull ? cc_site[(uint32_t)(tk & smask)] : 0u;
+  near_row_offer_bulk<4u>(q, kk, ss, cc_site_, SB, ulps, ln);
+  near_track(q, tk, ts, tk != ~0ull);
+  return wave_sum(lane < 3u ? (uint32_t)(sw >> 32) : 0u);
 }
 
 #ifndef PROP_TILE
diff --git a/protocol_amd/csrc/pm_stream.inc b/protocol_amd/csrc/pm_stream.inc
--- a/protocol_amd/csrc/pm_stream.inc
+++ b/protocol_amd/csrc/pm_stream.inc
@@ -1739,19 +1739,23 @@
   }
   return false;
 }
+template <bool PARTS = false>
 __device__ __forceinline__ bool stream_bitmap_sweep(const CarveArgs& p, const uint64_t* cfg64, uint32_t n, uint32_t* wl, uint32_t lane,
                                                     uint32_t s, bool shared, uint32_t ssite, const SeedGeo& sg, uint32_t SB,
-                                                    uint64_t ulps, NearRow& q, uint32_t& n_mine, BulkCtx& bulk, uint32_t ci, uint32_t ticket) {
+                                                    uint64_t ulps, NearRow& q, uint32_t& n_mine, BulkCtx& bulk, uint32_t ci, uint32_t ticket,
+                                                    uint32_t part = 0u, uint32_t np = 1u) {
   const auto freeg = G((const unsigned long long*)p.bits_scratch);
   const auto cfgb = G(cfg64);
-  const uint32_t lw = (n + 63u) >> 6;
+  const uint32_t lw_all = (n + 63u) >> 6;
+  const uint32_t lw = !PARTS ? lw_all : lw_all > part ? (lw_all - part + np - 1u) / np : 0u;
   uint32_t nb = 0u;
   SWEEP_PROF_DECL;
   const auto locg = G((const unsigned long long*)p.loc_g);
   const uint32_t sw = UNI(p.mode) != CARVE_MODE_MERGE ? s >> 6 : 0u;
   const unsigned long long s_below = UNI(p.mode) != CARVE_MODE_MERGE ? (1ull << (s & 63u)) - 1ull : 0ull;
-  auto word = [&](uint32_t j) -> unsigned long long {
-    if (j >= lw) return 0ull;
+  auto word = [&](uint32_t i) -> unsigned long long {
+    if (i >= lw) return 0ull;
+    const uint32_t j = !PARTS ? i : i * np + part;
     unsigned long long a = ld_ag(&freeg[j]) & cfgb[j];
     if (j <= sw) a &= ~(locg[j] & (j < sw ? ~0ull : s_below));
     return a;
@@ -1763,7 +1767,7 @@
     const uint32_t cw = (uint32_t)__popcll(a);
     const uint32_t incl = wave_incl_scan_u32(cw);
     uint32_t o = nb + incl - cw;
-    const uint32_t base = (j0 + lane) * 64u;
+    const uint32_t base = (!PARTS ? j0 + lane : (j0 + lane) * np + part) * 64u;
     for (; a; a &= a - 1ull) wl[o++] = base + (uint32_t)__builtin_ctzll(a);
     nb += (uint32_t)__builtin_amdgcn_readlane((int)incl, 63);
     PM_REC(if (bulk.rec_pass == 0) bulk.rec_pass = STREAM_CLOCK();)
@@ -1789,17 +1793,160 @@
   return false;
 }
 
+#ifndef STREAM_SHARED_MIN_CAND
+#define STREAM_SHARED_MIN_CAND 1024u
+#endif
+enum { SHR_ROW = 0u, SHR_SKIP = 1u, SHR_LEAVE = 2u, SHR_SPLIT = 3u };
+__device__ __forceinline__ uint32_t stream_wait_ticket(const CarveArgs& p, uint32_t n, uint32_t t, uint32_t lane, uint32_t& pay) {
+  const auto ctl = G(p.stream_ctl);
+  const auto sq = G((const unsigned long long*)p.stream_sq);
+  const uint32_t tag0 = UNI(p.stream_tag0);
+  uint32_t nap = 8u;
+  pay = 0u;
+  for (uint32_t spins = 0u;;) {
+    const unsigned long long g = ld_ag(&sq[t & (PM_STREAM_SQ - 1u)]);
+    if (UNI((uint32_t)(g >> 32)) == tag0 + t) {
+      pay = UNI((uint32_t)g);
+      break;
+    }
+    if ((spins & 255u) == 255u && UNI(ld_ag32(&ctl[SC_QUIT]))) return SHR_LEAVE;
+    if (nap >= 32u) __builtin_amdgcn_s_sleep(STREAM_NAP_LONG);
+    else if (nap >= 16u) __builtin_amdgcn_s_sleep(STREAM_NAP_LONG < 32 ? STREAM_NAP_LONG : 32);
+    else __builtin_amdgcn_s_sleep(STREAM_NAP_LONG < 16 ? STREAM_NAP_LONG : 16);
+    nap = nap < 32u ? nap << 1 : nap;
+    if (++spins > PM_STREAM_IDLE_SPINS) {
+      if (lane == 0u) atomicAdd(&p.stream_ctl[SC_GAVE_UP], 1u);
+      return SHR_LEAVE;
+    }
+  }
+  if (pay == 0xFFFFFFFFu) return SHR_LEAVE;
+  if ((pay & 0x3FFFFu) >= n || STREAM_DROPPED(UNI(ld_ag32(&ctl[SC_DROP])), (pay >> 18) & 63u, t)) return SHR_SKIP;
+  return SHR_ROW;
+}
+__device__ __forceinline__ void stream_deliver_row(const CarveArgs& p, const NearRow& q, uint32_t swept, uint32_t t, uint64_t t_seen, uint32_t SB,
+                                                   double TIE_BAND, uint32_t lane) {
+  const auto sq = G((const unsigned long long*)p.stream_sq);
+  const auto row_lo = G(p.stream_row_lo);
+  const auto row_hi = G(p.stream_row_hi);
+  const uint32_t tag0 = UNI(p.stream_tag0);
+  uint64_t mine;
+  const uint32_t meta = near_row_finish(p, q, true, PM_PROP_KMAX, SB, TIE_BAND, lane, &mine);
+  if (p.count_keys && lane == 0u) {
+    atomicAdd((unsigned long long*)&p.status->prop_keys, (unsigned long long)swept);
+    atomicAdd(&p.status->n_props, 1u);
+  }
+  if (__builtin_amdgcn_s_memtime() - t_seen > STREAM_LATE_ROW_TICKS) {
+    const unsigned long long g2 = ld_ag(&sq[t & (PM_STREAM_SQ - 1u)]);
+    if (UNI((uint32_t)(g2 >> 32)) != tag0 + t) return;
+  }
+  const size_t rb = (size_t)(t & (PM_STREAM_RQ - 1u)) * 64u + ((lane + 1u) & 63u);
+  const unsigned long long tagw = (unsigned long long)(tag0 + t) << 32;
+  st_ag(&row_hi[rb], tagw | (lane == 63u ? 0ull : (unsigned long long)(uint32_t)(mine >> 32)));
+  asm volatile("s_waitcnt vmcnt(0)" ::: "memory");
+  st_ag(&row_lo[rb], tagw | (lane == 63u ? (unsigned long long)meta : (unsigned long long)(uint32_t)mine));
+}
+__device__ __forceinline__ bool stream_proposer_shared(const CarveArgs& p, unsigned char* s_raw, uint32_t n, uint32_t SB, double TIE_BAND,
+                                                       uint64_t WINDOW_ULPS, uint32_t* wl, BulkCtx& bulk, uint32_t& t_given) {
+  static_assert((3u * NEAR_PART_U64 + 4u) * 8u <= STREAM_WL_WORDS * 4u, "they fit it");
+  const uint32_t lane = threadIdx.x & 63u, wave = threadIdx.x >> 6;
+  uint64_t* const parts = reinterpret_cast<uint64_t*>(s_raw) + size_t(CARVE_WAVES - 1u) * STREAM_WL_WORDS / 2u;
+  volatile uint32_t* const slots = reinterpret_cast<volatile uint32_t*>(parts + 3u * NEAR_PART_U64);
+  const bool by_length = UNI(p.stream_shared) >= 2u;
+  uint32_t ci_seen = PM_NONE;
+  bool long_seen = true;
+  const bool over = wave == 1u && G((const CarveStatus*)p.status)->state != CARVE_STATE_RUNNING;
+  uint32_t n_shared = 0u;
+  uint32_t t_claim = 0u;
+  if (wave == 1u && lane == 0u && !over) t_claim = atomicAdd(&p.stream_ctl[SC_CLAIM], 1u);
+  auto sweep = [&](uint32_t np, uint32_t t, uint32_t pay, uint32_t part, NearRow& q, uint32_t& swept) -> bool {
+    const uint32_t s = pay & 0x3FFFFu, ci = (pay >> 18) & 63u;
+    const uint64_t* cfg64 = p.cfgbits + (size_t)ci * p.bits_stride;
+    const uint32_t ssite = G(p.cc_site)[s];
+    const SeedGeo sg = {G(p.cc_lat)[s], G(p.cc_lon)[s], G(p.cc_cos)[s], G(p.cc_ux)[s], G(p.cc_uy)[s], G(p.cc_uz)[s]};
+    const bool shared = (ssite & 0x80000000u) != 0u;
+    q = NearRow{~0ull, ~0ull, ~0ull, ~0ull, ~0ull, 0xFFFFFFFFu};
+    uint32_t n_mine = 0;
+    bulk.seen = 0u;
+    PM_REC(bulk.rec_pass = bulk.rec_keys = 0;)
+    const bool let_be = stream_bitmap_sweep<true>(p, cfg64, n, wl, lane, s, shared, ssite, sg, SB, WINDOW_ULPS, q, n_mine, bulk, ci, t, part, np);
+    swept = wave_sum(n_mine);
+    return UNI(let_be);
+  };
+  for (uint32_t it = 0u;; ++it) {
+    volatile uint32_t* const slot = slots + (it & 1u) * 4u;
+    if (wave == 1u) {
+      const uint32_t t = UNI(t_claim);
+      uint32_t pay = 0u;
+      uint32_t what = over ? (uint32_t)SHR_LEAVE : stream_wait_ticket(p, n, t, lane, pay);
+      if (by_length && what == SHR_ROW) {
+        const uint32_t ci = (pay >> 18) & 63u;
+        if (ci != ci_seen) {
+          const auto freeg = G((const unsigned long long*)p.bits_scratch);
+          const auto cfgb = G(p.cfgbits + (size_t)ci * p.bits_stride);
+          uint32_t cnt = 0u;
+          for (uint32_t j = lane; j < ((n + 63u) >> 6); j += 64u) cnt += (uint32_t)__popcll(ld_ag(&freeg[j]) & cfgb[j]);
+          ci_seen = ci;
+          long_seen = wave_sum(cnt) >= STREAM_SHARED_MIN_CAND;
+        }
+        if (!long_seen) what = SHR_SPLIT;
+      }
+      if (lane == 0u) {
+        slot[0] = what;
+        slot[1] = t;
+        slot[2] = pay;
+        slot[3] = 0u;
+      }
+    }
+    __syncthreads();
+    const uint32_t what = UNI(slot[0]), t = UNI(slot[1]), pay = UNI(slot[2]);
+    if (what == SHR_LEAVE || what == SHR_SPLIT) {
+      if (wave == 0u && lane == 0u && n_shared) atomicAdd(&p.status->stream_shared_rows, n_shared);
+      if (what == SHR_LEAVE) return false;
+      if (wave == 1u) t_given = t;
+      return true;
+    }
+    NearRow q;
+    uint32_t swept = 0u;
+    const uint64_t t_seen = __builtin_amdgcn_s_memtime();
+    if (wave == 1u && lane == 0u) t_claim = atomicAdd(&p.stream_ctl[SC_CLAIM], 1u);
+    if (what == SHR_SKIP) continue;
+    PM_PROF(const uint64_t bt0 = t_seen;)
+    PM_REC(const uint64_t rec_seen = STREAM_CLOCK();)
+    const bool let_be = sweep(4u, t, pay, wave, q, swept);
+    PM_PROF(const uint64_t bt_geo = bt0;)
+    if (wave != 0u) near_part_post(parts + (wave - 1u) * NEAR_PART_U64, q, swept, lane);
+    if (let_be && lane == 0u) slot[3] = 1u;
+    __syncthreads();
+    if (wave != 0u) continue;
+    if (UNI(slot[3])) {
+      if (lane == 0u) atomicAdd(&p.stream_ctl[SC_LET_BE], 1u);
+      continue;
+    }
+    swept += near_row_merge_parts(q, parts, p.cc_site, SB, WINDOW_ULPS, bulk.ln);
+    PM_PROF(const uint64_t bt1 = PM_TICKS();)
+    PM_REC(const uint64_t rec_swept = STREAM_CLOCK();)
+    stream_deliver_row(p, q, swept, t, t_seen, SB, TIE_BAND, lane);
+    n_shared += 1u;
+    PM_REC(const uint64_t rec_fin = STREAM_CLOCK();)
+    const uint32_t swept_l0 = lane == 0u ? swept : 0u;
+    (void)swept_l0;
+    PROP_REC_ROW(t, (uint32_t)SROW_BITMAP, swept_l0, rec_seen, bulk, rec_swept, rec_fin);
+    PROP_PROF_ROW(t, (uint32_t)SROW_BITMAP, q, swept_l0, bt0, bt_geo, bt1);
+  }
+}
+
 __device__ __forceinline__ void stream_proposer(const CarveArgs& p, unsigned char* s_raw) {
   const uint32_t lane = threadIdx.x & 63u, wave = threadIdx.x >> 6;
   if (wave >= PM_STREAM_PROP_WAVES) return;
   const auto st = G((const CarveStatus*)p.status);
-  if (st->state != CARVE_STATE_RUNNING) return;
   const uint32_t n = st->n_eligible;
+  const uint32_t cell_g = st->cell_g;
+  const bool share = PM_STREAM_PROP_WAVES == 4u && UNI(p.stream_shared) && (!cell_g || !p.prune_mode);
+  if (!share && st->state != CARVE_STATE_RUNNING) return;
   if (n == 0u || n > PM_CARVE_BIG_SLOTS) return;
   const uint32_t SB = n > PM_CARVE_SLOTS ? PM_CARVE_SLOT_BITS_BIG : PM_CARVE_SLOT_BITS;
   const double TIE_BAND = n > PM_CARVE_SLOTS ? PM_TIE_BAND_BIG : PM_TIE_BAND;
   const uint64_t WINDOW_ULPS = n > PM_CARVE_SLOTS ? (1ull << 25) : (1ull << 20);
-  const uint32_t cell_g = st->cell_g;
   static_assert(STREAM_WL_WORDS >= 2u * CELL_BUF, "the walk's buffer fits the sweep's");
   static_assert(size_t(CARVE_WAVES) * STREAM_WL_WORDS * 4u <= PM_STREAM_LDS_BYTES, "one candidate buffer per wave");
   uint32_t* wl = reinterpret_cast<uint32_t*>(s_raw) + wave * STREAM_WL_WORDS;
@@ -1811,10 +1958,17 @@
   static_assert(size_t(CARVE_WAVES) * STREAM_WL_WORDS * 4u + size_t(CARVE_WAVES) * NET_PACK_KEYS * 8u <= PM_STREAM_LDS_BYTES,
                 "a packing list per wave behind the buffers");
   BulkCtx bulk = {0u, lane_net(lane, reinterpret_cast<uint64_t*>(s_raw + size_t(CARVE_WAVES) * STREAM_WL_WORDS * 4u) + wave * NET_PACK_KEYS)};
+  uint32_t t_given = PM_NONE;
+  if (share) {
+    if (!stream_proposer_shared(p, s_raw, n, SB, TIE_BAND, WINDOW_ULPS, wl, bulk, t_given)) return;
+  }
   for (;;) {
-    uint32_t t = 0u;
-    if (lane == 0u) t = atomicAdd(&p.stream_ctl[SC_CLAIM], 1u);
-    t = UNI(t);
+    uint32_t t = UNI(t_given);
+    t_given = PM_NONE;
+    if (t == PM_NONE) {
+      if (lane == 0u) t = atomicAdd(&p.stream_ctl[SC_CLAIM], 1u);
+      t = UNI(t);
+    }
     unsigned long long g;
     uint32_t nap = 8u;
     for (uint32_t spins = 0u;;) {
@@ -2201,15 +2355,17 @@
   const CarveArgs& p = *pa;
   extern __shared__ __attribute__((aligned(16))) unsigned char s_raw[];
   const uint32_t lane = threadIdx.x & 63u, wave = threadIdx.x >> 6;
-  if (wave != 0u) return;
+  const bool wg_row = PM_ROWB(16u), four = PM_ROWB(32u);
+  if (wave >= (wg_row || four ? 4u : 1u)) return;
   const auto st = G((const CarveStatus*)p.status);
   const uint32_t n = st->n_eligible;
   if (n == 0u || n > PM_CARVE_BIG_SLOTS || s >= n) return;
   const uint32_t SB = n > PM_CARVE_SLOTS ? PM_CARVE_SLOT_BITS_BIG : PM_CARVE_SLOT_BITS;
   const double TIE_BAND = n > PM_CARVE_SLOTS ? PM_TIE_BAND_BIG : PM_TIE_BAND;
   const uint64_t WINDOW_ULPS = n > PM_CARVE_SLOTS ? (1ull << 25) : (1ull << 20);
-  uint32_t* wl = reinterpret_cast<uint32_t*>(s_raw);
-  BulkCtx bulk = {0u, lane_net(lane, reinterpret_cast<uint64_t*>(s_raw + size_t(CARVE_WAVES) * STREAM_WL_WORDS * 4u))};
+  uint32_t* wl = reinterpret_cast<uint32_t*>(s_raw) + wave * STREAM_WL_WORDS;
+  BulkCtx bulk = {0u, lane_net(lane, reinterpret_cast<uint64_t*>(s_raw + size_t(CARVE_WAVES) * STREAM_WL_WORDS * 4u) + wave * NET_PACK_KEYS)};
+  uint64_t* const parts = reinterpret_cast<uint64_t*>(s_raw) + size_t(CARVE_WAVES - 1u) * STREAM_WL_WORDS / 2u;
   const uint64_t* cfg64 = p.cfgbits + (size_t)ci * p.bits_stride;
   unsigned long long t_all = 0, t_geo = 0, t_sweep = 0, t_fin = 0, check = 0;
   uint32_t swept = 0;
@@ -2223,21 +2379,31 @@
     bulk.seen = 0u;
     asm volatile("s_waitcnt vmcnt(0)" ::: "memory");
     const uint64_t t1 = __builtin_amdgcn_s_memtime();
-    (void)stream_bitmap_sweep(p, cfg64, n, wl, lane, s, shared, ssite, sg, SB, WINDOW_ULPS, q, n_mine, bulk, ci, 0x01FFFFF0u);
+    uint32_t others = 0u;
+    if (wg_row) {
+      (void)stream_bitmap_sweep<true>(p, cfg64, n, wl, lane, s, shared, ssite, sg, SB, WINDOW_ULPS, q, n_mine, bulk, ci, 0x01FFFFF0u, wave, 4u);
+      if (wave != 0u) near_part_post(parts + (wave - 1u) * NEAR_PART_U64, q, wave_sum(n_mine), lane);
+      __syncthreads();
+      if (wave == 0u) others = near_row_merge_parts(q, parts, p.cc_site, SB, WINDOW_ULPS, bulk.ln);
+    } else {
+      (void)stream_bitmap_sweep(p, cfg64, n, wl, lane, s, shared, ssite, sg, SB, WINDOW_ULPS, q, n_mine, bulk, ci, 0x01FFFFF0u);
+    }
     const uint64_t t2 = __builtin_amdgcn_s_memtime();
     uint64_t mine = q.m1;
-    const uint32_t meta = PM_ROWB(1u) ? 0u : near_row_finish(p, q, true, PM_PROP_KMAX, SB, TIE_BAND, lane, &mine);
+    const uint32_t meta = PM_ROWB(1u) || (wg_row && wave != 0u) ? 0u : near_row_finish(p, q, true, PM_PROP_KMAX, SB, TIE_BAND, lane, &mine);
+    if (wg_row || four) __syncthreads();
     const uint64_t t3 = __builtin_amdgcn_s_memtime() + (meta & 0u);
     t_all += t3 - t0;
     t_geo += t1 - t0;
     t_sweep += t2 - t1;
     t_fin += t3 - t2;
-    swept = wave_sum(n_mine);
+    swept = wave_sum(n_mine) + others;
     check = mine * (lane + 1u) + meta;
   }
   unsigned long long cs = check;
   for (uint32_t o = 32u; o; o >>= 1) cs += __shfl_xor(cs, o, 64);
-  if (lane == 0u) {
+  if (lane == 0u && wave == 0u) {
+    out[8] = (G(p.cc_site)[s] & 0x80000000u) ? 1ull : 0ull;
     out[0] = t_all;
     out[1] = reps;
     out[2] = swept;
diff --git a/protocol_amd/engine.py b/protocol_amd/engine.py
--- a/protocol_amd/engine.py
+++ b/protocol_amd/engine.py
@@ -671,14 +671,15 @@
         L = lib()
         L.pm_debug_carve_prof.argtypes = [C.c_void_p, C.POINTER(C.c_ulonglong), C.c_uint32]
         L.pm_debug_carve_prof.restype = C.c_int32
-        out = (C.c_ulonglong * 98)()
-        check(L.pm_debug_carve_prof(self._h, out, 98))
+        out = (C.c_ulonglong * 99)()
+        check(L.pm_debug_carve_prof(self._h, out, 99))
         w = [int(v) for v in out[32:56]]
         return {"why": w[:8], "batches": w[8], "void_launches": w[9], "pruned_batches": w[10], "prune_fallbacks": w[11],
                 "cell_g": w[12], "n_indexed": w[13],
                 "stream": w[14], "stream_tickets": w[15], "stream_timeouts": w[16], "stream_switches": w[17],
                 "stream_listed": w[18], "stream_wgs": w[19], "stream_aborts": w[20], "slow_steps": w[21],
-                "stream_pre_used": w[22], "stream_pre_lost": w[23], "stream_refreshes": int(out[97])}
+                "stream_pre_used": w[22], "stream_pre_lost": w[23], "stream_refreshes": int(out[97]),
+                "stream_shared_rows": int(out[98])}
 
     def debug_prune_mode(self, mode: int):
         L = lib()
```
